# NVlabs/implicit_depth

Hardware: AMD Instinct MI355X
Metric: Mpoints/sec implicit-MLP query, 240x320x64 samples; depth L1 vs ref (higher is better)
Workload: dtype f32

## Files before the change

### implicit_depth_amd/csrc/lidf_api.hip

```cpp
#include <string.h>
#include <stdlib.h>

#include "lidf_launch.h"
#include "lidf_hip.h"

#define LIDF_API extern "C" __attribute__((visibility("default")))
#define CHECK_HIP(x)                       \
    do {                                   \
        if ((x) != hipSuccess) return LIDF_ERR_HIP; \
    } while (0)

static inline size_t align_up(size_t v, size_t a) { return (v + a - 1) / a * a; }
static size_t linex_stream_bytes(int k);

static hipError_t zero_words(void* a, size_t words_a, void* b, size_t words_b, hipStream_t st) {
    float* ptrs[2] = {(float*)a, (float*)b};
    const long long cnt[2] = {(long long)words_a, (long long)words_b};
    return lidf_launch_zero_segments(ptrs, cnt, 2, st);
}

static thread_local const LidfPackGuardState* tl_guard = nullptr;
struct GuardScope {
    explicit GuardScope(const LidfPackGuardState* g) { tl_guard = g; }
    ~GuardScope() { tl_guard = nullptr; }
};
static inline StreamLayout guarded(StreamLayout lay) {
    lay.guard = tl_guard;
    return lay;
}
static thread_local PackJobs* tl_jobs = nullptr;
static hipError_t flush_jobs(PackJobs& j, hipStream_t st) {
    const hipError_t e = lidf_launch_pack_multi(j, st);
    j.n = 0;
    return e;
}
static hipError_t pack_stream(const StreamLayout& lay, const NetW& n0, const NetW& n1, const L1Map& m,
                              float* stream, float* aux, hipStream_t st) {
    if (!tl_jobs) return lidf_launch_pack(guarded(lay), n0, n1, m, stream, aux, st);
    if (tl_jobs->n == LIDF_PACK_JOBS) {
        const hipError_t e = flush_jobs(*tl_jobs, st);
        if (e != hipSuccess) return e;
    }
    PackJob& k = tl_jobs->job[tl_jobs->n++];
    k.lay = guarded(lay); k.n0 = n0; k.n1 = n1; k.m = m; k.stream = stream; k.aux = aux;
    return hipSuccess;
}
struct JobScope {
    PackJobs jobs;
    JobScope() { jobs.n = 0; tl_jobs = &jobs; }
    ~JobScope() { tl_jobs = nullptr; }
};
static inline unsigned long long salt_mix(unsigned long long h, unsigned long long v) {
    h ^= v + 0x9E3779B97F4A7C15ull + (h << 6) + (h >> 2);
    h = (h ^ (h >> 30)) * 0xBF58476D1CE4E5B9ull;
    return h ^ (h >> 27);
}

static int cu_count(int* out) {
    int dev = 0;
    if (hipGetDevice(&dev) != hipSuccess) return LIDF_ERR_HIP;
    if (hipDeviceGetAttribute(out, hipDeviceAttributeMultiprocessorCount, dev) != hipSuccess)
        return LIDF_ERR_HIP;
    if (*out <= 0) *out = 256;
    return LIDF_OK;
}

static hipError_t zero_decoder_grads(const LidfDecoderGrads* g, int ld1, int is_ief, hipStream_t st) {
    float* const p[10] = {g->w1, g->b1, g->w2, g->b2, g->w3, g->b3, g->w4, g->b4,
                          is_ief ? g->wenc : nullptr, is_ief ? g->benc : nullptr};
    const long long c[10] = {(long long)LIDF_H1 * ld1, LIDF_H1, (long long)LIDF_H2 * LIDF_H1, LIDF_H2,
                             (long long)LIDF_H3 * LIDF_H2, LIDF_H3, LIDF_H3, 1, 16, 16};
    return lidf_launch_zero_segments(p, c, 10, st);
}

static int check_decoder(const LidfDecoder* d) {
    if (!d) return LIDF_OK;
    if (!d->w1 || !d->b1 || !d->w2 || !d->b2 || !d->w3 || !d->b3 || !d->w4 || !d->b4)
        return LIDF_ERR_BAD_ARG;
    if (d->is_ief && (!d->wenc || !d->benc || d->n_iter < 1 || d->n_iter > 64))
        return LIDF_ERR_BAD_ARG;
    return LIDF_OK;
}

static NetW to_netw(const LidfDecoder* d, int dcore) {
    NetW n;
    n.w1 = d->w1; n.b1 = d->b1; n.w2 = d->w2; n.b2 = d->b2;
    n.w3 = d->w3; n.b3 = d->b3; n.w4 = d->w4; n.b4 = d->b4;
    n.wenc = d->wenc; n.benc = d->benc;
    n.is_ief = d->is_ief ? 1 : 0;
    n.dcore = dcore;
    n.ld1 = dcore + (d->is_ief ? 16 : 0);
    return n;
}

static L1Map rows_map(int n0, int c0, int n1, int c1, int add_bias) {
    L1Map m = {};
    m.n0 = n0; m.c0 = c0; m.n1 = n1; m.c1 = c1;
    m.D = n0 + n1;
    m.KQ1 = (m.D + 1 + 7) / 8;
    m.add_bias = add_bias;
    m.nt = 8;
    m.nout = 256;
    return m;
}

static void fill_net_args(PointsArgs& a, int i, const LidfDecoder* d, float* out, int is_offset) {
    a.npass[i] = d->is_ief ? d->n_iter : 1;
    a.init[i] = d->is_ief ? d->init_offset : 0.f;
    a.sigmoid[i] = d->use_sigmoid;
    a.out[i] = out;
    a.is_offset[i] = is_offset;
}

LIDF_API int lidf_version(void) { return LIDF_ABI_VERSION; }

LIDF_API const char* lidf_strerror(int status) {
    switch (status) {
        case LIDF_OK: return "ok";
        case LIDF_ERR_BAD_ARG: return "lidf_hip: bad argument (null pointer, negative size or inconsistent sizes)";
        case LIDF_ERR_UNSUPPORTED: return "lidf_hip: unsupported dimension";
        case LIDF_ERR_WORKSPACE: return "lidf_hip: workspace too small";
        case LIDF_ERR_HIP: return "lidf_hip: HIP runtime error";
        default: return "lidf_hip: unknown status";
    }
}

LIDF_API int lidf_embed_f32(const float* x, int64_t n, int multires, float* out,
                              lidf_stream_t stream) {
    if (n < 0 || multires < 0 || multires > 16) return LIDF_ERR_BAD_ARG;
    if (n == 0) return LIDF_OK;
    if (!x || !out) return LIDF_ERR_BAD_ARG;
    CHECK_HIP(lidf_launch_embed(x, n, multires, out, (hipStream_t)stream));
    return LIDF_OK;
}

LIDF_API size_t lidf_decoders_workspace_bytes(int64_t n, int d) {
    (void)n;
    if (d <= 0) return 0;
    L1Map m = rows_map(d, 0, 0, 0, 1);
    StreamLayout lay = lidf_make_layout(2, LIDF_MODE_ROWS, m);
    const size_t hs = (size_t)lidf_make_layout_rows_h(2, d, 0).total * 4;
    const size_t fs = (size_t)lay.total * 4;
    return align_up(fs > hs ? fs : hs, 256) + align_up(2 * LIDF_AUX_FLOATS * 4, 256);
}

static int decoders_impl(const float* inp, int64_t n, int d, int64_t ld_inp, const LidfDecoder* prob,
                         const LidfDecoder* off, float* out_prob, float* out_off, void* workspace,
                         size_t workspace_bytes, int precision, lidf_stream_t stream,
                         const int* n_dev = nullptr);

LIDF_API int lidf_decoders_f32(const float* inp, int64_t n, int d, int64_t ld_inp,
                                 const LidfDecoder* prob, const LidfDecoder* off, float* out_prob,
                                 float* out_off, void* workspace, size_t workspace_bytes,
                                 lidf_stream_t stream) {
    return decoders_impl(inp, n, d, ld_inp, prob, off, out_prob, out_off, workspace, workspace_bytes,
// ... 2410 lines not shown
    if (!(voxpart_ready && pack_mode == 2) && (rc = run_linex(L, (float*)s_vox, cus, st, pack_mode))) return rc;
    if (make_raypart || pack_mode == 1) {
        LinEx Lr = {};
        Lr.w = off->w1; Lr.b = nullptr; Lr.ldw = ld1; Lr.nout = LIDF_H1;
        Lr.k = 128; Lr.c0 = 128;
        Lr.k1 = Ed; Lr.c1 = 256 + E;
        Lr.dcore = D;
        Lr.X = rayfeat; Lr.ldx = 128 + Ed; Lr.n = R; Lr.out = raypart; Lr.ld_out = LIDF_H1;
        Lr.n_dev = R_dev;
        if ((rc = run_linex(Lr, (float*)s_ray, cus, st, pack_mode))) return rc;
    }
    char* s16 = s_chain + chain_stream_bytes(D - 128);
    float* aux16 = (float*)(s16 + align_up(ief16_stream_bytes(3 + 6 * 16), 256));
    if (pack_mode != 2) {
        StreamLayout lay = {};
        lay.nets = 1; lay.mode = LIDF_MODE_IEF16;
        lay.total = (int)(ief16_stream_bytes(E) / 4);
        L1Map m16 = {};
        m16.n0 = E; m16.c0 = 256;
        const NetW nw = to_netw(off, D);
        CHECK_HIP(pack_stream(lay, nw, nw, m16, (float*)s16, aux16, st));
    }
    if (!use_ief16() || pack_mode == 1) {
        if (ev_rows && ev_rows[0] && pack_mode != 1) CHECK_HIP(hipEventRecord((hipEvent_t)ev_rows[0], st));
        rc = run_chain_train(off, D, rows_map(E, 256, 0, 0, 0), inp_embed ? inp_embed + 256 : nullptr, D, R,
                             end_voxel, nullptr, voxpart, raypart, nullptr, nullptr, out, s_chain, cus, st,
                             LIDF_MODE_ROWS_GATHER, pack_mode, R_dev);
        if (!rc && ev_rows && ev_rows[1] && pack_mode != 1) CHECK_HIP(hipEventRecord((hipEvent_t)ev_rows[1], st));
        return rc;
    }
    if (R <= 0) return LIDF_OK;
    if (ev_rows && ev_rows[0]) CHECK_HIP(hipEventRecord((hipEvent_t)ev_rows[0], st));
    Ief16Args ia = {};
    ia.stream = (const float*)s16; ia.aux = aux16; ia.KQ = (E + 15) / 16; ia.E = E;
    ia.n = R; ia.n_dev = R_dev;
    ia.X = inp_embed + 256; ia.ldx = D;
    ia.vox = end_voxel; ia.voxpart = voxpart; ia.raypart = raypart;
    ia.npass = off->is_ief ? off->n_iter : 1;
    ia.init = off->is_ief ? off->init_offset : 0.f;
    ia.sigmoid = off->use_sigmoid;
    ia.out = out;
    CHECK_HIP(lidf_launch_ief16(ia, cus, st));
    if (ev_rows && ev_rows[1]) CHECK_HIP(hipEventRecord((hipEvent_t)ev_rows[1], st));
    return LIDF_OK;
}

LIDF_API size_t lidf_refine_pack_bytes(int32_t multires, int32_t multires_views) {
    if (multires < 0 || multires > 16 || multires_views < 0 || multires_views > 16) return 0;
    return align_up(refine_fact_bytes(refine_D(multires, multires_views)), 256);
}

LIDF_API int lidf_refine_pack_f32(const LidfDecoder* off, int32_t multires, int32_t multires_views,
                                    void* packed, size_t packed_bytes, lidf_stream_t stream) {
    if (!off) return LIDF_ERR_BAD_ARG;
    int rc;
    if ((rc = check_decoder(off))) return rc;
    const size_t need = lidf_refine_pack_bytes(multires, multires_views);
    if (!need) return LIDF_ERR_UNSUPPORTED;
    if (!packed || packed_bytes < need) return LIDF_ERR_WORKSPACE;
    JobScope js;
    if ((rc = refine_pack_into(off, multires, multires_views, (char*)packed, (hipStream_t)stream))) return rc;
    CHECK_HIP(flush_jobs(js.jobs, (hipStream_t)stream));
    return LIDF_OK;
}

LIDF_API int lidf_refine_pack_guarded_f32(const LidfDecoder* off, int32_t multires,
                                            int32_t multires_views, void* packed, size_t packed_bytes,
                                            void* guard, lidf_stream_t stream) {
    if (!off || !guard) return LIDF_ERR_BAD_ARG;
    int rc;
    if ((rc = check_decoder(off))) return rc;
    const size_t need = lidf_refine_pack_bytes(multires, multires_views);
    if (!need) return LIDF_ERR_UNSUPPORTED;
    if (!packed || packed_bytes < need) return LIDF_ERR_WORKSPACE;
    const float* ptrs[LIDF_FP_MAX_SEGS];
    long long cnt[LIDF_FP_MAX_SEGS];
    const int k = decoder_segs(off, refine_D(multires, multires_views), ptrs, cnt, 0);
    return guarded_pack(ptrs, cnt, k, refine_salt(off, multires, multires_views), guard, (hipStream_t)stream, [&] {
        return lidf_refine_pack_f32(off, multires, multires_views, packed, packed_bytes, stream);
    });
}

struct TrainWs {
    size_t stream, dz1, dz2, dz3, S, goff, wg, chain, small, total;
};
static TrainWs train_ws(int64_t n, int d) {
    TrainWs w;
    const size_t N = (size_t)(n > 0 ? n : 1);
    size_t o = 0;
    const int kmax = d > 256 ? d : 256;
    w.stream = o; o += linex_stream_bytes(kmax);
    w.dz1 = o;    o += align_up(N * LIDF_H1 * 4, 256);
    w.dz2 = o;    o += align_up(N * LIDF_H2 * 4, 256);
    w.dz3 = o;    o += align_up(N * LIDF_H3 * 4, 256);
    w.S = o;      o += align_up(N * LIDF_H1 * 4, 256);
    w.goff = o;   o += align_up(N * 4, 256);
    w.wg = o;     o += align_up(WG_SCRATCH_FLOATS * 4, 256);
    w.chain = o;  o += chain_stream_bytes(d);
    w.small = o;  o += 512 * 4;
    w.total = o;
    return w;
}
LIDF_API size_t lidf_decoder_train_workspace_bytes(int64_t n, int32_t d) { return train_ws(n, d).total; }

static inline const unsigned* act_m1(const float* pass, int64_t n) { return (const unsigned*)(pass + (size_t)n * LIDF_ACT_M1); }
static inline const unsigned* act_m2(const float* pass, int64_t n) { return (const unsigned*)(pass + (size_t)n * LIDF_ACT_M2); }
static inline const float* act_h1(const float* act, int64_t n, int k) { return act + (size_t)k * n * ACT_ROW_FLOATS; }

LIDF_API int lidf_decoder_forward_train_f32(const float* inp, int64_t n, int32_t d, int64_t ld_inp,
                                              const LidfDecoder* dec, float* out, float* act,
                                              void* workspace, size_t workspace_bytes,
                                              lidf_stream_t stream) {
    if (n < 0 || d <= 0 || ld_inp < d || !dec) return LIDF_ERR_BAD_ARG;
    int rc;
    if ((rc = check_decoder(dec))) return rc;
    if (n == 0) return LIDF_OK;
    if (!inp || !out || !act) return LIDF_ERR_BAD_ARG;
    const TrainWs w = train_ws(n, d);
    if (!workspace || workspace_bytes < w.total) return LIDF_ERR_WORKSPACE;
    hipStream_t st = (hipStream_t)stream;
    float* sbuf = (float*)((char*)workspace + w.stream);
    int cus;
    if ((rc = cu_count(&cus))) return rc;
    const int npass = dec->is_ief ? dec->n_iter : 1;
    const int ld1 = d + (dec->is_ief ? 16 : 0);
    float* pre = act + (size_t)npass * n * ACT_ROW_FLOATS;
    (void)ld1; (void)sbuf;
    if ((rc = run_chain_train(dec, d, rows_map(d, 0, 0, 0, 1), inp, ld_inp, n, nullptr, nullptr, nullptr,
                              nullptr, act, pre, out, (char*)workspace + w.chain, cus, st)))
        return rc;
    return LIDF_OK;
}

static int decoder_backward_core(const float* inp, int64_t n, int32_t d, int64_t ld_inp, const LidfDecoder* dec,
                                 const float* act, const float* g_out, const LidfDecoderGrads* grads, char* ws,
                                 const TrainWs& w, int cus, hipStream_t st, float** S_out) {
    const int npass = dec->is_ief ? dec->n_iter : 1;
    const int ld1 = d + (dec->is_ief ? 16 : 0);
    float* sbuf = (float*)(ws + w.stream);
    float* dz1 = (float*)(ws + w.dz1);
    float* dz2 = (float*)(ws + w.dz2);
    float* dz3 = (float*)(ws + w.dz3);
    float* goff = (float*)(ws + w.goff);
    float* wgs = (float*)(ws + w.wg);
    const float* pre = act + (size_t)npass * n * ACT_ROW_FLOATS;
    float* S = (float*)(ws + w.S);
    float* small = (float*)(ws + w.small);
    CHECK_HIP(hipMemsetAsync(small, 0, 512 * 4, st));
    CHECK_HIP(lidf_launch_out_act(pre, n, dec->use_sigmoid, nullptr, g_out, goff, st));
    CHECK_HIP(lidf_launch_pack_dgrad(dec->w3, dec->w2, sbuf, st));
    if (npass == 1) S = dz1;
    for (int k = npass - 1; k >= 0; --k) {
        const float* h1 = act_h1(act, n, k);
        const float* h2 = h1 + (size_t)n * LIDF_H1;
        const float* h3 = h2 + (size_t)n * LIDF_H2;
        const float* offin = h3 + (size_t)n * LIDF_H3;
        CHECK_HIP(lidf_launch_l4_backward(goff, h3, dec->w4, 0.02f, n, dz3, grads->w4, grads->b4, wgs, st));
        CHECK_HIP(lidf_launch_wgrad(dz3, LIDF_H3, LIDF_H3, h2, LIDF_H2, LIDF_H2, n, grads->w3, LIDF_H2, grads->b3, wgs, WG_SCRATCH_FLOATS, st));
        const bool first_pass_short = dec->is_ief && npass > 1 && k == 0;
        float* dz1k = (k == npass - 1 || first_pass_short) ? S : dz1;
        CHECK_HIP(lidf_launch_dgrad_chain(nullptr, nullptr, dz3, act_m2(h1, n), act_m1(h1, n), n, 0.02f, dz2, dz1k,
                                          first_pass_short ? 1 : 0, sbuf, cus, st));
        CHECK_HIP(lidf_launch_wgrad(dz2, LIDF_H2, LIDF_H2, h1, LIDF_H1, LIDF_H1, n, grads->w2, LIDF_H1, grads->b2, wgs, WG_SCRATCH_FLOATS, st));
        if (dec->is_ief && !first_pass_short)
            CHECK_HIP(lidf_launch_ief_tail(dz1k, offin, dec->w1 + d, ld1, dec->wenc, dec->benc, n,
                                           k == npass - 1 ? 0 : 2, S, goff, grads->w1 + d, grads->wenc,
                                           grads->benc, npass > 1 ? small : nullptr, wgs, st));
    }
    CHECK_HIP(lidf_launch_wgrad(S, LIDF_H1, LIDF_H1, inp, ld_inp, d, n, grads->w1, ld1, grads->b1, wgs, WG_SCRATCH_FLOATS, st));
    if (dec->is_ief && npass > 1)
        CHECK_HIP(lidf_launch_ief_first_pass(grads->b1, small, dec->init_offset, dec->w1 + d, ld1, dec->wenc,
                                             dec->benc, grads->w1 + d, grads->wenc, grads->benc, st));
    *S_out = S;
    return LIDF_OK;
}

static int check_decoder_grads(const LidfDecoder* dec, const LidfDecoderGrads* grads) {
    if (!grads->w1 || !grads->b1 || !grads->w2 || !grads->b2 || !grads->w3 || !grads->b3 ||
        !grads->w4 || !grads->b4 || (dec->is_ief && (!grads->wenc || !grads->benc)))
        return LIDF_ERR_BAD_ARG;
    return LIDF_OK;
}

static int decoder_input_grad(const float* S, const LidfDecoder* dec, const float* S2, const LidfDecoder* dec2,
                              int64_t n, int32_t d, float* d_inp, int64_t ld_dinp, float* sbuf, int cus,
                              hipStream_t st) {
    LinEx L = {};
    L.n = n; L.transposed = 1; L.mask_slope = 0.02f;
    const int ld1 = d + (dec->is_ief ? 16 : 0);
    bool xcol = d % 32 == 1 && d > 32 && n > 16 * 128;
    if (xcol) {
        const int t = (d - 1) / 32, l = (t + 7) / 8;
        if ((t + l - 1) / l >= 8) xcol = false;
    }
    const int dt = xcol ? d - 1 : d;
    const int tiles = (dt + 31) / 32, launches = (tiles + 7) / 8, per = (tiles + launches - 1) / launches;
    for (int c0 = 0; c0 < dt; c0 += 32 * per) {
        int cols = dt - c0 < 32 * per ? dt - c0 : 32 * per;
        L.xcol = 0;
        if (xcol && c0 + cols == dt) { cols += 1; L.xcol = 1; }
        L.w = dec->w1 + c0; L.ldw = ld1; L.nout = cols; L.k = LIDF_H1; L.X = S; L.ldx = LIDF_H1;
        if (S2) {
            L.X2 = S2; L.ldx2 = LIDF_H1; L.k2 = LIDF_H1;
            L.w_2 = dec2->w1 + c0; L.ldw_2 = d + (dec2->is_ief ? 16 : 0);
        }
        L.out = d_inp + c0; L.ld_out = ld_dinp; L.accumulate = 0;
        int rc;
        if ((rc = run_linex(L, sbuf, cus, st))) return rc;
    }
    return LIDF_OK;
}

LIDF_API int lidf_decoder_backward_f32(const float* inp, int64_t n, int32_t d, int64_t ld_inp,
                                         const LidfDecoder* dec, const float* act,
                                         const float* g_out, float* d_inp, int64_t ld_dinp,
                                         const LidfDecoderGrads* grads, void* workspace,
                                         size_t workspace_bytes, lidf_stream_t stream) {
    if (n < 0 || d <= 0 || ld_inp < d || !dec || !grads) return LIDF_ERR_BAD_ARG;
    int rc;
    if ((rc = check_decoder(dec))) return rc;
    if ((rc = check_decoder_grads(dec, grads))) return rc;
    if (d_inp && ld_dinp < d) return LIDF_ERR_BAD_ARG;
    hipStream_t st = (hipStream_t)stream;
    CHECK_HIP(zero_decoder_grads(grads, d + (dec->is_ief ? 16 : 0), dec->is_ief, st));
    if (n == 0) return LIDF_OK;
    if (!inp || !act || !g_out) return LIDF_ERR_BAD_ARG;
    const TrainWs w = train_ws(n, d);
    if (!workspace || workspace_bytes < w.total) return LIDF_ERR_WORKSPACE;
    char* ws = (char*)workspace;
    int cus;
    if ((rc = cu_count(&cus))) return rc;
    float* S = nullptr;
    if ((rc = decoder_backward_core(inp, n, d, ld_inp, dec, act, g_out, grads, ws, w, cus, st, &S))) return rc;
    if (d_inp) return decoder_input_grad(S, dec, nullptr, nullptr, n, d, d_inp, ld_dinp, (float*)(ws + w.stream), cus, st);
    return LIDF_OK;
}

LIDF_API size_t lidf_decoder_pair_workspace_bytes(int64_t n, int32_t d) {
    return 2 * align_up(train_ws(n, d).total, 256) + linex_stream_bytes(2 * LIDF_H1);
}
LIDF_API size_t lidf_decoder_pair_workspace_offset(int64_t n, int32_t d, int32_t which) {
    return (size_t)(which ? 1 : 0) * align_up(train_ws(n, d).total, 256);
}

LIDF_API int lidf_decoder_pair_backward_f32(const float* inp, int64_t n, int32_t d, int64_t ld_inp,
                                              const LidfDecoder* prob, const LidfDecoder* off,
                                              const float* act_prob, const float* act_off,
                                              const float* g_prob, const float* g_off, float* d_inp,
                                              int64_t ld_dinp, const LidfDecoderGrads* grads_prob,
                                              const LidfDecoderGrads* grads_off, void* workspace,
                                              size_t workspace_bytes, lidf_stream_t stream) {
    if (n < 0 || d <= 0 || ld_inp < d || !prob || !off || !grads_prob || !grads_off) return LIDF_ERR_BAD_ARG;
    int rc;
    if ((rc = check_decoder(prob)) || (rc = check_decoder(off))) return rc;
    if ((rc = check_decoder_grads(prob, grads_prob)) || (rc = check_decoder_grads(off, grads_off))) return rc;
    if (d_inp && ld_dinp < d) return LIDF_ERR_BAD_ARG;
    hipStream_t st = (hipStream_t)stream;
    CHECK_HIP(zero_decoder_grads(grads_prob, d + (prob->is_ief ? 16 : 0), prob->is_ief, st));
    CHECK_HIP(zero_decoder_grads(grads_off, d + (off->is_ief ? 16 : 0), off->is_ief, st));
    if (n == 0) return LIDF_OK;
    if (!inp || !act_prob || !act_off || !g_prob || !g_off) return LIDF_ERR_BAD_ARG;
    const TrainWs w = train_ws(n, d);
    const size_t one = align_up(w.total, 256);
    if (!workspace || workspace_bytes < lidf_decoder_pair_workspace_bytes(n, d)) return LIDF_ERR_WORKSPACE;
    char* ws = (char*)workspace;
    int cus;
    if ((rc = cu_count(&cus))) return rc;
    float *Sp = nullptr, *So = nullptr;
    if ((rc = decoder_backward_core(inp, n, d, ld_inp, prob, act_prob, g_prob, grads_prob, ws, w, cus, st, &Sp))) return rc;
    if ((rc = decoder_backward_core(inp, n, d, ld_inp, off, act_off, g_off, grads_off, ws + one, w, cus, st, &So))) return rc;
    if (d_inp) return decoder_input_grad(Sp, prob, So, off, n, d, d_inp, ld_dinp, (float*)(ws + 2 * one), cus, st);
    return LIDF_OK;
}

LIDF_API int lidf_build_rows_f32(const int32_t* pair_ray, const int32_t* pair_vox,
                                   const float* pair_t, const float* ray_dir,
                                   const float* vox_center, int32_t pos_rel, const float* vox_feat,
                                   const float* rayfeat, int32_t multires, int32_t multires_views,
                                   int64_t n_pairs, float* rows, lidf_stream_t stream) {
    if (n_pairs < 0 || multires < 0 || multires > 16 || multires_views < 0 || multires_views > 16)
        return LIDF_ERR_BAD_ARG;
    if (n_pairs == 0) return LIDF_OK;
    if (!pair_ray || !pair_vox || !pair_t || !ray_dir || !vox_feat || !rayfeat || !rows)
        return LIDF_ERR_BAD_ARG;
    if (pos_rel && !vox_center) return LIDF_ERR_BAD_ARG;
    const int Ed = 3 + 6 * multires_views;
    CHECK_HIP(lidf_launch_build_rows(pair_ray, pair_vox, pair_t, ray_dir, vox_center, pos_rel,
                                     vox_feat, rayfeat, 128 + Ed, multires, Ed, n_pairs, rows,
                                     query_D(multires, multires_views), (hipStream_t)stream));
    return LIDF_OK;
}

LIDF_API int lidf_rows_backward_f32(const float* d_rows, const int32_t* pair_off,
                                      const int32_t* pair_vox, int64_t n_rays, int64_t n_pairs,
                                      int64_t n_vox, int32_t multires, int32_t multires_views,
                                      float* d_vox_feat, float* d_rayfeat, lidf_stream_t stream) {
    if (n_pairs < 0 || n_rays < 0 || n_vox < 0 || multires < 0 || multires > 16 ||
        multires_views < 0 || multires_views > 16)
        return LIDF_ERR_BAD_ARG;
    hipStream_t st = (hipStream_t)stream;
    const int E = 3 + 6 * multires, Ed = 3 + 6 * multires_views;
    if (d_vox_feat && n_vox > 0) CHECK_HIP(hipMemsetAsync(d_vox_feat, 0, (size_t)n_vox * 128 * 4, st));
    if (n_rays == 0) return LIDF_OK;
    if (!pair_off || (n_pairs > 0 && (!d_rows || !pair_vox))) return LIDF_ERR_BAD_ARG;
    CHECK_HIP(lidf_launch_rows_backward(d_rows, query_D(multires, multires_views), 2 * E, pair_off, pair_vox, n_rays,
                                        n_pairs, Ed, d_vox_feat, d_rayfeat, 128 + Ed, st));
    return LIDF_OK;
}

LIDF_API int lidf_ray_features_backward_f32(const float* d_rayfeat, const int32_t* ray_pix,
                                              const int32_t* ray_bid, int64_t n_rays, int32_t batch,
                                              int32_t height, int32_t width, int32_t roi_inp_bbox,
                                              int32_t multires_views, float* d_feat_grid,
                                              void* workspace, size_t workspace_bytes,
                                              lidf_stream_t stream) {
    if (n_rays < 0 || batch <= 0 || height <= 0 || width <= 0 || !d_feat_grid) return LIDF_ERR_BAD_ARG;
    hipStream_t st = (hipStream_t)stream;
    CHECK_HIP(hipMemsetAsync(d_feat_grid, 0, (size_t)batch * 32 * height * width * 4, st));
    if (n_rays == 0) return LIDF_OK;
    if (!d_rayfeat || !ray_pix || !ray_bid) return LIDF_ERR_BAD_ARG;
    const size_t need = (size_t)batch * 128 * height * width * 4;
    const size_t need2 = need + (size_t)batch * height * width * 4;
    float* gimg = (workspace && workspace_bytes >= need) ? (float*)workspace : nullptr;
    int* pix_rays = (workspace && workspace_bytes >= need2) ? (int*)((char*)workspace + need) : nullptr;
    CHECK_HIP(lidf_launch_rayfeat_backward(d_rayfeat, 128 + 3 + 6 * multires_views, ray_pix, ray_bid,
                                           n_rays, roi_inp_bbox / 2, batch, height, width, d_feat_grid,
                                           gimg, pix_rays, st));
    return LIDF_OK;
}

LIDF_API int lidf_pe_rows_f32(const int32_t* pair_ray, const int32_t* pair_vox, const float* pair_t,
                                const float* ray_dir, const float* vox_center, int32_t pos_rel,
                                int32_t multires, int64_t n_pairs, float* pe, lidf_stream_t stream) {
    if (n_pairs < 0 || multires < 0 || multires > 16) return LIDF_ERR_BAD_ARG;
    if (n_pairs == 0) return LIDF_OK;
    if (!pair_ray || !pair_vox || !pair_t || !ray_dir || !pe || (pos_rel && !vox_center))
        return LIDF_ERR_BAD_ARG;
    if (n_pairs * 2 * (3 + 6 * multires) > 0x7fffffffLL * 256) return LIDF_ERR_UNSUPPORTED;
    CHECK_HIP(lidf_launch_pe_rows(pair_ray, pair_vox, pair_t, ray_dir, vox_center, pos_rel, multires,
                                  n_pairs, pe, (hipStream_t)stream));
    return LIDF_OK;
}

static inline size_t qact_pass(int64_t P) { return (size_t)P * ACT_ROW_FLOATS; }

LIDF_API size_t lidf_query_decoder_act_floats(int64_t n_pairs, int64_t n_rays, int64_t n_vox,
                                                int32_t n_pass) {
    if (n_pairs < 0 || n_rays < 0 || n_vox < 0 || n_pass <= 0) return 0;
    return (size_t)(n_vox + n_rays) * LIDF_H1 + (size_t)n_pass * qact_pass(n_pairs) + (size_t)n_pairs;
}

struct QTrainWs {
    size_t stream, dz1, dz2, dz3, S, goff, dvox, dray, wg, seg, seg_bytes, chain, small, total;
};
static QTrainWs qtrain_ws(int64_t P, int64_t R, int64_t V) {
    QTrainWs w;
    const size_t N = (size_t)(P > 0 ? P : 1);
    size_t o = 0;
    w.stream = o; o += linex_stream_bytes(256);
    w.dz1 = o;    o += align_up(N * LIDF_H1 * 4, 256);
    w.dz2 = o;    o += align_up(N * LIDF_H2 * 4, 256);
    w.dz3 = o;    o += align_up(N * LIDF_H3 * 4, 256);
    w.S = o;      o += align_up(N * LIDF_H1 * 4, 256);
    w.goff = o;   o += align_up(N * 4, 256);
    w.dvox = o;   o += align_up((size_t)(V > 0 ? V : 1) * LIDF_H1 * 4, 256);
    w.dray = o;   o += align_up((size_t)(R > 0 ? R : 1) * LIDF_H1 * 4, 256);
    w.wg = o;     o += align_up(WG_SCRATCH_FLOATS * 4, 256);
    w.seg_bytes = lidf_seg_sum_idx_ws_bytes(P, V);
    w.seg = o;    o += align_up(w.seg_bytes, 256);
    w.chain = o;  o += chain_stream_bytes(2 * (3 + 6 * 16));
    w.small = o;  o += 512 * 4;
    w.total = o;
    return w;
}
LIDF_API size_t lidf_query_decoder_workspace_bytes(int64_t n_pairs, int64_t n_rays, int64_t n_vox) {
    return qtrain_ws(n_pairs, n_rays, n_vox).total;
}

static int check_qtrain(const LidfQueryTrainArgs* q) {
    if (!q || !q->dec) return LIDF_ERR_BAD_ARG;
    if (q->n_pairs < 0 || q->n_rays < 0 || q->n_vox < 0) return LIDF_ERR_BAD_ARG;
    if (q->multires < 0 || q->multires > 16 || q->multires_views < 0 || q->multires_views > 16)
        return LIDF_ERR_BAD_ARG;
    if (q->n_pairs > 0 && (!q->pair_off || !q->pair_ray || !q->pair_vox || !q->pe || !q->vox_feat ||
                           !q->rayfeat || q->n_rays == 0 || q->n_vox == 0))
        return LIDF_ERR_BAD_ARG;
    return check_decoder(q->dec);
}

static int qdec_forward_impl(const LidfQueryTrainArgs* q, int E2, float* out, float* voxpart, float* raypart,
                             float* passes, float* pre, float* s_vox, float* s_ray, char* s_chain, int cus,
                             hipStream_t st, int pack_mode = 0, int parts = 7, int pe_ld = 0) {
    int rc;
    const int64_t P = q->n_pairs, R = q->n_rays, V = q->n_vox;
    const LidfDecoder* dec = q->dec;
    const int Ed = 3 + 6 * q->multires_views;
    const int D = 256 + E2 + Ed, ld1 = D + (dec->is_ief ? 16 : 0);
    LinEx L = {};
    if (parts & 1) {
        L.w = dec->w1; L.b = dec->b1; L.ldw = ld1; L.nout = LIDF_H1; L.k = 128; L.dcore = D;
        L.ief = dec->is_ief ? dec : nullptr;
        L.X = q->vox_feat; L.ldx = 128; L.n = V; L.out = voxpart; L.ld_out = LIDF_H1;
        if ((rc = run_linex(L, s_vox, cus, st, pack_mode))) return rc;
    }
    if (parts & 2) {
        L = {};
        L.w = dec->w1; L.ldw = ld1; L.nout = LIDF_H1; L.k = 128; L.c0 = 128; L.k1 = Ed; L.c1 = 256 + E2;
        L.X = q->rayfeat; L.ldx = 128 + Ed; L.n = R; L.out = raypart; L.ld_out = LIDF_H1;
        if ((rc = run_linex(L, s_ray, cus, st, pack_mode))) return rc;
    }
    if (parts & 4) {
        if ((rc = run_chain_train(dec, D, rows_map(E2, 256, 0, 0, 0), q->pe, pe_ld ? pe_ld : E2, P, q->pair_vox,
                                  q->pair_ray, voxpart, raypart, passes, pre, out, s_chain, cus, st, LIDF_MODE_TRAIN,
                                  pack_mode)))
            return rc;
    }
    return LIDF_OK;
}

LIDF_API int lidf_query_decoder_forward_train_f32(const LidfQueryTrainArgs* q, float* out, float* act,
                                                    void* workspace, size_t workspace_bytes,
                                                    lidf_stream_t stream) {
    int rc;
    if ((rc = check_qtrain(q))) return rc;
    const int64_t P = q->n_pairs, R = q->n_rays, V = q->n_vox;
    if (P == 0) return LIDF_OK;
    if (!out || !act) return LIDF_ERR_BAD_ARG;
    const QTrainWs w = qtrain_ws(P, R, V);
    if (!workspace || workspace_bytes < w.total) return LIDF_ERR_WORKSPACE;
    hipStream_t st = (hipStream_t)stream;
    float* sbuf = (float*)((char*)workspace + w.stream);
    int cus;
    if ((rc = cu_count(&cus))) return rc;
    const LidfDecoder* dec = q->dec;
    const int E2 = 2 * (3 + 6 * q->multires);
    const int npass = dec->is_ief ? dec->n_iter : 1;
    float* voxpart = act;
    float* raypart = voxpart + (size_t)V * LIDF_H1;
    float* passes = raypart + (size_t)R * LIDF_H1;
    float* pre = passes + (size_t)npass * qact_pass(P);
    return qdec_forward_impl(q, E2, out, voxpart, raypart, passes, pre, sbuf, sbuf, (char*)workspace + w.chain,
                             cus, st);
}

LIDF_API size_t lidf_query_forward_train_workspace_bytes(int64_t n_rays, int64_t n_vox) {
    return lidf_query_workspace_bytes(n_rays, n_vox, 0);
}

LIDF_API int lidf_query_forward_train_f32(const LidfQueryTrainArgs* q, const LidfDecoder* offset_dec,
                                            const float* pair_t, const float* ray_dir,
                                            const float* vox_center, int32_t pos_rel, float* out_prob,
                                            float* out_off, float* act_prob, float* act_off,
                                            void* workspace, size_t workspace_bytes,
                                            lidf_stream_t stream) {
    int rc;
    if ((rc = check_qtrain(q))) return rc;
    if ((rc = check_decoder(offset_dec))) return rc;
    const int64_t P = q->n_pairs, R = q->n_rays, V = q->n_vox;
    if (P > 0x7fffffffLL || R > 0x15555555LL) return LIDF_ERR_UNSUPPORTED;
    const int L = q->multires, Lv = q->multires_views;
    if ((rc = check_query_model(q->dec, offset_dec, L, Lv, LIDF_PRECISION_F32))) return rc;
    if (P == 0) return LIDF_OK;
    if (!pair_t || !ray_dir || !out_prob || !out_off || !act_prob || !act_off || (pos_rel && !vox_center))
        return LIDF_ERR_BAD_ARG;
    const QueryWs w = query_ws(R, V, L, Lv);
    if (!workspace || workspace_bytes < w.total) return LIDF_ERR_WORKSPACE;
    hipStream_t st = (hipStream_t)stream;
    char* ws = (char*)workspace;
    const QueryPlan p = query_plan(L, Lv, LIDF_PRECISION_F32);
    if ((rc = pack_query_weights(q->dec, offset_dec, p, ws, st))) return rc;
    int cus;
    if ((rc = cu_count(&cus))) return rc;
    CHECK_HIP(lidf_launch_l1only_pair(
        l1_table_args(p, L1_RAY, q->rayfeat, R, nullptr, (float*)(ws + w.raypart), ws, w),
        l1_table_args(p, L1_VOX, q->vox_feat, V, nullptr, (float*)(ws + w.voxpart), ws, w), nullptr, cus, st));
    PointsArgs a = points_args(p, ws, ws, w, P, q->pair_ray, q->pair_vox, pair_t, ray_dir, vox_center, pos_rel,
                               0.f, 0.f, 0.f);
    fill_net_args(a, 0, q->dec, out_prob, 0);
    fill_net_args(a, 1, offset_dec, out_off, 1);
    const LidfDecoder* decs[2] = {q->dec, offset_dec};
    float* acts[2] = {act_prob, act_off};
    for (int i = 0; i < 2; ++i) {
        const int np = decs[i]->is_ief ? decs[i]->n_iter : 1;
        a.tr_passes[i] = acts[i] + (size_t)(V + R) * LIDF_H1;
        a.tr_pre[i] = a.tr_passes[i] + (size_t)np * qact_pass(P);
    }
    a.tr_pass_floats = (long long)qact_pass(P);
    const long long nt = (P + 127) / 128;
    CHECK_HIP(lidf_launch_points(LIDF_MODE_FUSED, a, (int)(nt < cus ? nt : cus), st));
    return LIDF_OK;
}

LIDF_API int lidf_query_forward_train_selected_f32(const LidfQueryTrainArgs* q, const LidfDecoder* offset_dec,
                                                     const float* pair_t, const float* ray_dir,
                                                     const float* vox_center, int32_t pos_rel, float offset_range0,
                                                     float offset_range1, float part_size,
                                                     const int64_t* max_pair_id_in, float* out_prob, float* softmax,
                                                     int64_t* max_pair_id, float* pred_offset, float* pair_pred_pos,
                                                     float* pred_pos, float* act_prob, float* act_off_rows,
                                                     void* workspace, size_t workspace_bytes, lidf_stream_t stream) {
    int rc;
    if ((rc = check_qtrain(q))) return rc;
    if ((rc = check_decoder(offset_dec))) return rc;
    const int64_t P = q->n_pairs, R = q->n_rays, V = q->n_vox;
    if (P > 0x7fffffffLL || R > 0x15555555LL) return LIDF_ERR_UNSUPPORTED;
    const int L = q->multires, Lv = q->multires_views;
    if ((rc = check_query_model(q->dec, offset_dec, L, Lv, LIDF_PRECISION_F32))) return rc;
    if (R == 0) return LIDF_OK;
    if (!max_pair_id || !pred_pos) return LIDF_ERR_BAD_ARG;
    hipStream_t st = (hipStream_t)stream;
    if (P == 0) {
        CHECK_HIP(lidf_launch_ray_reduce_dev(nullptr, nullptr, q->pair_off, R, 0, nullptr, nullptr, nullptr, nullptr, 0,
                                             nullptr, (long long*)max_pair_id, pred_pos, nullptr, st, nullptr, nullptr,
                                             nullptr, nullptr, nullptr));
        return LIDF_OK;
    }
    if (!pair_t || !ray_dir || !out_prob || !softmax || !pred_offset || !pair_pred_pos || !act_prob || !act_off_rows ||
        (pos_rel && !vox_center))
        return LIDF_ERR_BAD_ARG;
    const QueryWs w = query_ws(R, V, L, Lv);
    if (!workspace || workspace_bytes < w.total) return LIDF_ERR_WORKSPACE;
    char* ws = (char*)workspace;
    const QueryPlan p = query_plan(L, Lv, LIDF_PRECISION_F32);
    if ((rc = pack_query_weights(q->dec, offset_dec, p, ws, st))) return rc;
    int cus;
    if ((rc = cu_count(&cus))) return rc;
    CHECK_HIP(lidf_launch_l1only_pair(
        l1_table_args(p, L1_RAY, q->rayfeat, R, nullptr, (float*)(ws + w.raypart), ws, w),
        l1_table_args(p, L1_VOX, q->vox_feat, V, nullptr, (float*)(ws + w.voxpart), ws, w), nullptr, cus, st));
    PointsArgs a = points_args(p, ws, ws, w, P, q->pair_ray, q->pair_vox, pair_t, ray_dir, vox_center, pos_rel,
                               offset_range0, offset_range1, part_size);
    a.nets = 1; a.part_ld = 512; a.part_off = 0;
    fill_net_args(a, 0, q->dec, out_prob, 0);
    a.tr_passes[0] = act_prob + (size_t)(V + R) * LIDF_H1;
    a.tr_pre[0] = a.tr_passes[0] + qact_pass(P);
    a.tr_pass_floats = (long long)qact_pass(P);
    const long long nt = (P + 127) / 128;
    CHECK_HIP(lidf_launch_points(LIDF_MODE_FUSED, a, (int)(nt < cus ? nt : cus), st));
    const SelList sl = sel_list(ws + w.sel, R);
    const bool given = max_pair_id_in != nullptr;
    CHECK_HIP(lidf_launch_ray_reduce_dev(out_prob, nullptr, q->pair_off, R, P, nullptr, nullptr, nullptr, nullptr, 0,
                                         softmax, (long long*)max_pair_id, nullptr, nullptr, st, q->pair_vox, pair_t,
                                         given ? nullptr : sl.ray, sl.vox, sl.t));
    if (given)
        CHECK_HIP(lidf_launch_sel_from_ids((const long long*)max_pair_id_in, q->pair_vox, pair_t, R, P, sl.ray, sl.vox,
                                           sl.t, st));
    const int npo = offset_dec->is_ief ? offset_dec->n_iter : 1;
    PointsArgs ao = offset_on_list(a, p, offset_dec, sl, R);
    ao.tr_passes[0] = act_off_rows + (size_t)(V + R) * LIDF_H1;
    ao.tr_pre[0] = ao.tr_passes[0] + (size_t)npo * qact_pass(R);
    ao.tr_pass_floats = (long long)qact_pass(R);
    const long long ntr = (R + 127) / 128;
    CHECK_HIP(lidf_launch_points(LIDF_MODE_FUSED, ao, (int)(ntr < cus ? ntr : cus), st));
    CHECK_HIP(lidf_launch_selected_finish((const long long*)(given ? max_pair_id_in : max_pair_id), sl.off, sl.pos, R, P,
                                          nullptr, nullptr, nullptr, nullptr, 0, pred_offset, pair_pred_pos, pred_pos,
                                          nullptr, st));
    return LIDF_OK;
}

struct QdecBwd {
    int E2;
    bool zero_grads;
    float* S_keep;
    float* d_pe;
    float *s_dvox, *s_dpe;
    int pack_mode;
    const float* s_dgrad;
    bool goff_ready;
    const float* l1rows;
    int l1_ld, l1_cols, l1_c0;
    const int *ss_perm, *ss_vstart, *ss_first;
    long long ss_row0, ss_n;
    float* ss_partial;
};
static int qdec_backward_impl(const LidfQueryTrainArgs* q, const QdecBwd& o, const float* passes, const float* pre,
                              const float* g_out, float* d_vox_feat, float* d_rayfeat, int accumulate_inputs,
                              const LidfDecoderGrads* grads, char* ws, const QTrainWs& w, int cus, hipStream_t st) {
    int rc;
    const LidfDecoder* dec = q->dec;
    const int64_t P = q->n_pairs, R = q->n_rays, V = q->n_vox;
    const int E2 = o.E2, Ed = 3 + 6 * q->multires_views;
    const int D = 256 + E2 + Ed, ld1 = D + (dec->is_ief ? 16 : 0);
    const int npass = dec->is_ief ? dec->n_iter : 1;
    float* sbuf = (float*)(ws + w.stream);
    float* dz1 = (float*)(ws + w.dz1);
    float* dz2 = (float*)(ws + w.dz2);
    float* dz3 = (float*)(ws + w.dz3);
    float* S = o.S_keep ? o.S_keep : (float*)(ws + w.S);
    float* goff = (float*)(ws + w.goff);
    float* wgs = (float*)(ws + w.wg);
    float* dvox = (float*)(ws + w.dvox);
    float* dray = (float*)(ws + w.dray);
    float* small = (float*)(ws + w.small);
    CHECK_HIP(hipMemsetAsync(small, 0, 512 * 4, st));
    if (!o.goff_ready) CHECK_HIP(lidf_launch_out_act(pre, P, dec->use_sigmoid, nullptr, g_out, goff, st));
    const float* dgs = o.s_dgrad;
    if (!dgs) {
        CHECK_HIP(lidf_launch_pack_dgrad(dec->w3, dec->w2, sbuf, st));
        dgs = sbuf;
    }
    for (int k = npass - 1; k >= 0; --k) {
        const float* h1 = passes + (size_t)k * qact_pass(P);
        const float* h2 = h1 + (size_t)P * LIDF_H1;
        const float* h3 = h2 + (size_t)P * LIDF_H2;
        const float* offin = h3 + (size_t)P * LIDF_H3;
        CHECK_HIP(lidf_launch_l4_backward(goff, h3, dec->w4, 0.02f, P, dz3, grads->w4, grads->b4, wgs, st));
        CHECK_HIP(lidf_launch_wgrad(dz3, LIDF_H3, LIDF_H3, h2, LIDF_H2, LIDF_H2, P, grads->w3, LIDF_H2, grads->b3, wgs, WG_SCRATCH_FLOATS, st));
        if (npass == 1) {
            if (o.S_keep) dz1 = S;
            else S = dz1;
        }
        const bool first_pass_short = dec->is_ief && npass > 1 && k == 0;
        float* dz1k = (k == npass - 1 || first_pass_short) ? S : dz1;
        CHECK_HIP(lidf_launch_dgrad_chain(nullptr, nullptr, dz3, act_m2(h1, P), act_m1(h1, P), P, 0.02f, dz2, dz1k,
                                          first_pass_short ? 1 : 0, (float*)dgs, cus, st));
        CHECK_HIP(lidf_launch_wgrad(dz2, LIDF_H2, LIDF_H2, h1, LIDF_H1, LIDF_H1, P, grads->w2, LIDF_H1, grads->b2, wgs, WG_SCRATCH_FLOATS, st));
        if (!first_pass_short)
            CHECK_HIP(lidf_launch_ief_tail(dz1k, offin, dec->is_ief ? dec->w1 + D : nullptr, ld1, dec->wenc,
                                           dec->benc, P, k == npass - 1 ? 0 : 2, S, goff,
                                           grads->w1 + D, grads->wenc, grads->benc,
                                           dec->is_ief && npass > 1 ? small : nullptr, wgs, st));
    }
    const bool short_first = dec->is_ief && npass > 1;
    if (o.l1rows)
        CHECK_HIP(lidf_launch_wgrad(S, LIDF_H1, LIDF_H1, o.l1rows, o.l1_ld, o.l1_cols, P, grads->w1 + o.l1_c0, ld1,
                                    short_first ? small + 256 : nullptr, wgs, WG_SCRATCH_FLOATS, st));
    else
        CHECK_HIP(lidf_launch_wgrad(S, LIDF_H1, LIDF_H1, q->pe, E2, E2, P, grads->w1 + 256, ld1,
                                    short_first ? small + 256 : nullptr, wgs, WG_SCRATCH_FLOATS, st));
    if (short_first)
        CHECK_HIP(lidf_launch_ief_first_pass(small + 256, small, dec->init_offset, dec->w1 + D, ld1,
                                             dec->wenc, dec->benc, grads->w1 + D, grads->wenc,
                                             grads->benc, st));
    if (o.ss_perm)
        CHECK_HIP(lidf_launch_pnet_gather_segsum(S, o.ss_perm, o.ss_row0, o.ss_vstart, o.ss_first, V, o.ss_n,
                                                 o.ss_partial, dvox, st));
    else
        CHECK_HIP(lidf_launch_seg_sum_idx(S, q->pair_vox, P, V, dvox, w.seg_bytes ? ws + w.seg : nullptr,
                                          w.seg_bytes, st));
    CHECK_HIP(lidf_launch_wgrad(dvox, LIDF_H1, LIDF_H1, q->vox_feat, 128, 128, V, grads->w1, ld1, grads->b1, wgs, WG_SCRATCH_FLOATS, st));
    if (!o.S_keep) {
        CHECK_HIP(lidf_launch_seg_sum_ray(S, LIDF_H1, q->pair_off, R, dray, st));
        CHECK_HIP(lidf_launch_wgrad(dray, LIDF_H1, LIDF_H1, q->rayfeat, 128 + Ed, 128, R, grads->w1 + 128, ld1, nullptr, wgs, WG_SCRATCH_FLOATS, st));
        CHECK_HIP(lidf_launch_wgrad(dray, LIDF_H1, LIDF_H1, q->rayfeat + 128, 128 + Ed, Ed, R, grads->w1 + 256 + E2, ld1, nullptr, wgs, WG_SCRATCH_FLOATS, st));
    }
    LinEx L = {};
    L.transposed = 1; L.ldw = ld1; L.k = LIDF_H1; L.ldx = LIDF_H1; L.accumulate = accumulate_inputs ? 1 : 0;
    if (d_vox_feat) {
        L.w = dec->w1; L.nout = 128; L.X = dvox; L.n = V; L.out = d_vox_feat; L.ld_out = 128;
        if ((rc = run_linex(L, o.s_dvox ? o.s_dvox : sbuf, cus, st, o.s_dvox ? o.pack_mode : 0))) return rc;
    }
    if (o.d_pe) {
        L.w = dec->w1 + 256; L.nout = E2; L.X = S; L.n = P; L.out = o.d_pe; L.ld_out = E2; L.accumulate = 0;
        if ((rc = run_linex(L, o.s_dpe ? o.s_dpe : sbuf, cus, st, o.s_dpe ? o.pack_mode : 0))) return rc;
        L.accumulate = accumulate_inputs ? 1 : 0;
    }
    if (d_rayfeat && !o.S_keep) {
        L.w = dec->w1 + 128; L.nout = 128; L.X = dray; L.n = R; L.out = d_rayfeat; L.ld_out = 128 + Ed;
        if ((rc = run_linex(L, sbuf, cus, st))) return rc;
        L.w = dec->w1 + 256 + E2; L.nout = Ed; L.out = d_rayfeat + 128;
        if ((rc = run_linex(L, sbuf, cus, st))) return rc;
    }
    return LIDF_OK;
}

LIDF_API int lidf_query_decoder_backward_f32(const LidfQueryTrainArgs* q, const float* act,
                                               const float* g_out, float* d_vox_feat,
                                               float* d_rayfeat, int32_t accumulate_inputs,
                                               const LidfDecoderGrads* grads, void* workspace,
                                               size_t workspace_bytes, lidf_stream_t stream) {
    int rc;
    if ((rc = check_qtrain(q))) return rc;
    if (!grads) return LIDF_ERR_BAD_ARG;
    const LidfDecoder* dec = q->dec;
    if (!grads->w1 || !grads->b1 || !grads->w2 || !grads->b2 || !grads->w3 || !grads->b3 ||
        !grads->w4 || !grads->b4 || (dec->is_ief && (!grads->wenc || !grads->benc)))
        return LIDF_ERR_BAD_ARG;
    const int64_t P = q->n_pairs, R = q->n_rays, V = q->n_vox;
    hipStream_t st = (hipStream_t)stream;
    const int E2 = 2 * (3 + 6 * q->multires), Ed = 3 + 6 * q->multires_views;
    const int D = 256 + E2 + Ed, ld1 = D + (dec->is_ief ? 16 : 0);
    const int npass = dec->is_ief ? dec->n_iter : 1;
    CHECK_HIP(zero_decoder_grads(grads, ld1, dec->is_ief, st));
    if (!accumulate_inputs) {
        if (d_vox_feat && V > 0) CHECK_HIP(hipMemsetAsync(d_vox_feat, 0, (size_t)V * 128 * 4, st));
        if (d_rayfeat && R > 0) CHECK_HIP(hipMemsetAsync(d_rayfeat, 0, (size_t)R * (128 + Ed) * 4, st));
    }
    if (P == 0) return LIDF_OK;
    if (!act || !g_out) return LIDF_ERR_BAD_ARG;
    const QTrainWs w = qtrain_ws(P, R, V);
    if (!workspace || workspace_bytes < w.total) return LIDF_ERR_WORKSPACE;
    int cus;
    if ((rc = cu_count(&cus))) return rc;
    const float* voxpart = act;
    const float* raypart = voxpart + (size_t)V * LIDF_H1;
    const float* passes = raypart + (size_t)R * LIDF_H1;
    const float* pre = passes + (size_t)npass * qact_pass(P);
    QdecBwd o = {};
    o.E2 = E2; o.zero_grads = true;
    return qdec_backward_impl(q, o, passes, pre, g_out, d_vox_feat, d_rayfeat, accumulate_inputs, grads,
                              (char*)workspace, w, cus, st);
}

struct QRowsWs { size_t pvox, poff, g, pe, act, inner, total; QTrainWs w; };
static QRowsWs qrows_ws(int64_t R, int64_t V, int E2, int npass) {
    QRowsWs l;
    const size_t N = (size_t)(R > 0 ? R : 1);
    size_t o = 0;
    l.pvox = o;  o += align_up(N * 4, 256);
    l.poff = o;  o += align_up((N + 1) * 4, 256);
    l.g = o;     o += align_up(N * 4, 256);
    l.pe = o;    o += align_up(N * (size_t)E2 * 4, 256);
    l.act = o;   o += align_up(((size_t)npass * qact_pass((int64_t)N) + N) * 4, 256);
    l.w = qtrain_ws(R, R, V);
    l.inner = o; o += l.w.total;
    l.total = o;
    return l;
}
LIDF_API size_t lidf_query_decoder_rows_workspace_bytes(int64_t n_rays, int64_t n_vox, int32_t multires,
                                                          int32_t n_pass) {
    if (n_rays < 0 || n_vox < 0 || multires < 0 || multires > 16 || n_pass <= 0) return 0;
    return qrows_ws(n_rays, n_vox, 2 * (3 + 6 * multires), n_pass).total;
}
LIDF_API int lidf_query_decoder_backward_rows_f32(const LidfQueryTrainArgs* q, const float* act, int32_t act_is_rows,
                                                    const int64_t* rows, const float* g_pred_pos,
                                                    const float* g_offset_rows, const float* ray_dir, float scale,
                                                    float* d_vox_feat,
                                                    float* d_rayfeat, int32_t accumulate_inputs,
                                                    const LidfDecoderGrads* grads, void* workspace,
                                                    size_t workspace_bytes, lidf_stream_t stream) {
    int rc;
    if ((rc = check_qtrain(q))) return rc;
    if (!grads) return LIDF_ERR_BAD_ARG;
    const LidfDecoder* dec = q->dec;
    if (!grads->w1 || !grads->b1 || !grads->w2 || !grads->b2 || !grads->w3 || !grads->b3 ||
        !grads->w4 || !grads->b4 || (dec->is_ief && (!grads->wenc || !grads->benc)))
        return LIDF_ERR_BAD_ARG;
    const int64_t P = q->n_pairs, R = q->n_rays, V = q->n_vox;
    hipStream_t st = (hipStream_t)stream;
    const int E2 = 2 * (3 + 6 * q->multires), Ed = 3 + 6 * q->multires_views;
    const int D = 256 + E2 + Ed, ld1 = D + (dec->is_ief ? 16 : 0);
    const int npass = dec->is_ief ? dec->n_iter : 1;
    CHECK_HIP(zero_decoder_grads(grads, ld1, dec->is_ief, st));
    if (!accumulate_inputs) {
        if (d_vox_feat && V > 0) CHECK_HIP(hipMemsetAsync(d_vox_feat, 0, (size_t)V * 128 * 4, st));
        if (d_rayfeat && R > 0) CHECK_HIP(hipMemsetAsync(d_rayfeat, 0, (size_t)R * (128 + Ed) * 4, st));
    }
    if (P == 0 || R == 0) return LIDF_OK;
    if (!act || !rows || !ray_dir) return LIDF_ERR_BAD_ARG;
    const QRowsWs l = qrows_ws(R, V, E2, npass);
    if (!workspace || workspace_bytes < l.total) return LIDF_ERR_WORKSPACE;
    int cus;
    if ((rc = cu_count(&cus))) return rc;
    char* ws = (char*)workspace;
    int* pvox = (int*)(ws + l.pvox);
    int* poff = (int*)(ws + l.poff);
    float* g = (float*)(ws + l.g);
    float* pe = (float*)(ws + l.pe);
    const float* passes_src = act + (size_t)(V + R) * LIDF_H1;
    const float* passes = act_is_rows ? passes_src : (const float*)(ws + l.act);
    CHECK_HIP(lidf_launch_gather_sel_rows(act_is_rows ? nullptr : passes_src, P, npass, (const long long*)rows, R,
                                          q->pair_vox, q->pe, E2, g_pred_pos, g_offset_rows, ray_dir, scale,
                                          (float*)(ws + l.act), pvox, pe, g, poff, st));
    LidfQueryTrainArgs qc = *q;
    qc.n_pairs = R;
    qc.pair_off = poff; qc.pair_ray = poff; qc.pair_vox = pvox; qc.pe = pe;
    QdecBwd o = {};
    o.E2 = E2; o.zero_grads = true;
    return qdec_backward_impl(&qc, o, passes, passes + (size_t)npass * qact_pass(R), g, d_vox_feat, d_rayfeat,
                              accumulate_inputs, grads, ws + l.inner, l.w, cus, st);
}

LIDF_API int lidf_query_tail_f32(const float* pred_offset, const float* pred_prob,
                                   const int32_t* pair_off, const int32_t* pair_ray,
                                   const float* pair_t, const float* ray_dir, int64_t n_rays,
                                   int64_t n_pairs, float offset_range0, float offset_range1,
                                   float part_size, const int64_t* max_pair_id_in,
                                   float* pair_pred_pos, float* softmax, int64_t* max_pair_id,
                                   float* pred_pos, lidf_stream_t stream) {
    if (n_rays < 0 || n_pairs < 0) return LIDF_ERR_BAD_ARG;
    if (n_rays == 0) return LIDF_OK;
    if (!pair_off || (n_pairs > 0 && (!pred_offset || !pred_prob || !pair_ray || !pair_t || !ray_dir ||
                                      !pair_pred_pos)))
        return LIDF_ERR_BAD_ARG;
    hipStream_t st = (hipStream_t)stream;
    CHECK_HIP(lidf_launch_pair_pos(pred_offset, pair_ray, pair_t, ray_dir, n_pairs, offset_range0,
                                   offset_range1 - offset_range0, (float)1.7320508075688772,
                                   part_size, pair_pred_pos, st));
    CHECK_HIP(lidf_launch_ray_reduce(pred_prob, pair_pred_pos, pair_off, n_rays, n_pairs, nullptr,
                                     nullptr, 0, softmax, (long long*)max_pair_id,
                                     max_pair_id_in ? nullptr : pred_pos, nullptr, st));
    if (max_pair_id_in && pred_pos)
        CHECK_HIP(lidf_launch_ray_select(pair_pred_pos, (const long long*)max_pair_id_in, n_rays,
                                         n_pairs, pred_pos, st));
    return LIDF_OK;
}

LIDF_API int lidf_query_tail_backward_f32(const float* g_pair_pred_pos, const float* g_pred_pos,
                                            const int64_t* max_pair_id, const int32_t* pair_ray,
                                            const float* ray_dir, int64_t n_rays, int64_t n_pairs,
                                            float offset_range0, float offset_range1,
                                            float part_size, float* d_pred_offset,
                                            lidf_stream_t stream) {
    if (n_rays < 0 || n_pairs < 0) return LIDF_ERR_BAD_ARG;
    if (n_pairs == 0) return LIDF_OK;
    if (!pair_ray || !ray_dir || !d_pred_offset || (g_pred_pos && !max_pair_id)) return LIDF_ERR_BAD_ARG;
    const float k = (offset_range1 - offset_range0) * (float)1.7320508075688772 * part_size;
    CHECK_HIP(lidf_launch_pair_pos_backward(g_pair_pred_pos, g_pred_pos, (const long long*)max_pair_id,
                                            pair_ray, ray_dir, n_pairs, k, d_pred_offset,
                                            (hipStream_t)stream));
    return LIDF_OK;
}

LIDF_API int lidf_embed_backward_f32(const float* x, const float* g_out, int64_t n, int multires,
                                       float* d_x, lidf_stream_t stream) {
    if (n < 0 || multires < 0 || multires > 16) return LIDF_ERR_BAD_ARG;
    if (n == 0) return LIDF_OK;
    if (!x || !g_out || !d_x) return LIDF_ERR_BAD_ARG;
    CHECK_HIP(lidf_launch_embed_backward(x, g_out, n, multires, d_x, (hipStream_t)stream));
    return LIDF_OK;
}

struct PnetAct {
    size_t f1, f2, f4, f5, pool1, g1, pool2, out, arg1, arg2, total;
};
static PnetAct pnet_act(int64_t n, int64_t v) {
    PnetAct a;
    const size_t N = (size_t)(n > 0 ? n : 1), V = (size_t)(v > 0 ? v : 1);
    size_t o = 0;
    a.f1 = o; o += N * 32;
    a.f2 = o; o += N * 64;
    a.f4 = o; o += N * 128;
    a.f5 = o; o += N * 128;
// ... 492 lines not shown
```

### implicit_depth_amd/csrc/lidf_api_refine_train.inc

```

struct RtLay {
    size_t s_pnf[7], s_pnb[PNET_BWD_SLOTS], s_pnchain, s_pnbwd, s_vox, s_ray, s_chain, s_dvox, s_dpe, s_dgrad;
    size_t raypart, ray_idx, iter0, iter_bytes, total;
    size_t cur, end_voxel, pn_inp, pn_vox, pnact, pe, voxpart, passes, pre, off;
};
static RtLay rt_lay(int64_t R, int64_t Nv, int64_t V, int E, int npass, int T) {
    RtLay l;
    size_t o = 0;
    const int ks[7] = {6, 32, 64, 64, 64, 128, 128};
    const int nts[7] = {1, 2, 2, 4, 4, 4, 4};
    for (int i = 0; i < 7; ++i) { l.s_pnf[i] = o; o += lin_stream_bytes(ks[i], nts[i]); }
    for (int i = 0; i < PNET_BWD_SLOTS; ++i) { l.s_pnb[i] = o; o += linex_stream_bytes(PNET_BWD_SLOT_K[i]); }
    l.s_pnchain = o; o += align_up(lidf_pointnet_chain_stream_bytes(), 256);
    l.s_pnbwd = o;   o += align_up(PNETC_BWD_STREAM_BYTES, 256);
    l.s_vox = o;   o += linex_stream_bytes(128);
    l.s_ray = o;   o += linex_stream_bytes(REFINE_RAY_K);
    l.s_chain = o; o += chain_stream_bytes(3 + 6 * 16);
    l.s_dvox = o;  o += linex_stream_bytes(256);
    l.s_dpe = o;   o += linex_stream_bytes(256);
    l.s_dgrad = o; o += align_up(lidf_dgrad_stream_bytes(), 256);
    const size_t r = (size_t)(R > 0 ? R : 1), n = (size_t)(R + Nv > 0 ? R + Nv : 1), v = (size_t)(V > 0 ? V : 1);
    l.raypart = o; o += align_up(r * LIDF_H1 * 4, 256);
    l.ray_idx = o; o += align_up(r * 4, 256);
    l.iter0 = o;
// ... 89 lines not shown
    }
    if (nc > 0x7fffffffLL) return LIDF_ERR_UNSUPPORTED;
    cells->g.crop = q->grid_part;
    cells->g.B = q->batch;
    cells->coord = q->voxel_coord;
    cells->table = q->cell_table;
    cells->ready = q->cell_table_ready;
    return LIDF_OK;
}

static int rt_pack_transposed(const LidfDecoder* dec, int E, int Ed, float* s_dvox, float* s_dpe, int cus,
                              hipStream_t st) {
    int rc;
    const int D = 256 + E + Ed, ld1 = D + (dec->is_ief ? 16 : 0);
    LinEx L = {};
    L.transposed = 1; L.ldw = ld1; L.k = LIDF_H1; L.ldx = LIDF_H1;
    L.w = dec->w1; L.nout = 128; L.ld_out = 128;
    if ((rc = run_linex(L, s_dvox, cus, st, 1))) return rc;
    L.w = dec->w1 + 256; L.nout = E; L.ld_out = E;
    return run_linex(L, s_dpe, cus, st, 1);
}

static void rt_query_args(const LidfRefineArgs* q, const RtLay& l, char* it, char* act, LidfQueryTrainArgs* t) {
    *t = {};
    t->n_pairs = q->n_rays; t->n_rays = q->n_rays; t->n_vox = q->n_vox;
    t->pair_off = nullptr;
    t->pair_ray = (const int32_t*)(act + l.ray_idx);
    t->pair_vox = (const int32_t*)(it + l.end_voxel);
    t->pe = (const float*)(it + l.pe) + 128;
    t->multires = q->multires; t->multires_views = q->multires_views;
    const int64_t n = q->n_rays + q->n_valid;
    t->vox_feat = pnetc_ok(n, q->n_vox) ? (const float*)(it + l.pnact + pnetc_act(n, q->n_vox).out)
                                        : (const float*)(it + l.pnact) + pnet_act(n, q->n_vox).out;
    t->rayfeat = q->rayfeat;
    t->dec = q->off;
}

LIDF_API int lidf_refine_train_forward_f32(const LidfRefineArgs* q, int32_t forward_times, void* act_v,
                                             size_t act_bytes, lidf_stream_t stream) {
    int rc, cus;
    const int T = forward_times;
    if ((rc = rt_check(q, T))) return rc;
    const int64_t R = q->n_rays, Nv = q->n_valid, V = q->n_vox, P = q->n_pairs, n = R + Nv;
    if (R == 0) return LIDF_OK;
    const LidfDecoder* dec = q->off;
    const int E = 3 + 6 * q->multires, Ed = 3 + 6 * q->multires_views;
    const int npass = dec->is_ief ? dec->n_iter : 1;
    const RtLay l = rt_lay(R, Nv, V, E, npass, T);
    const RtWs w = rt_ws(R, Nv, V, E);
    if (!act_v || act_bytes < l.total) return LIDF_ERR_WORKSPACE;
    if (!q->workspace || q->workspace_bytes < w.total) return LIDF_ERR_WORKSPACE;
    CellLookup cells;
    if ((rc = rt_cells(q, &cells))) return rc;
    if ((rc = cu_count(&cus))) return rc;
    hipStream_t st = (hipStream_t)stream;
    char* act = (char*)act_v;
    char* ws = (char*)q->workspace;
    const bool chain = pnetc_ok(n, V);
    float* pnf[7];
    float* pnb[PNET_BWD_SLOTS];
    for (int i = 0; i < 7; ++i) pnf[i] = (float*)(act + l.s_pnf[i]);
    for (int i = 0; i < PNET_BWD_SLOTS; ++i) pnb[i] = (float*)(act + l.s_pnb[i]);
    float* raypart = (float*)(act + l.raypart);
    int* ray_idx = (int*)(act + l.ray_idx);
    LidfQueryTrainArgs t;
    rt_query_args(q, l, act + l.iter0, act, &t);
    {
        JobScope js;
        if (chain)
            rc = pnetc_pack(q->pnet, (float*)(act + l.s_pnchain), pnf, (float*)(act + l.s_pnbwd), cus, st);
        else
            rc = pointnet_train_forward_impl(q->pnet, nullptr, nullptr, 0, 0, nullptr,
                                             (float*)(act + l.iter0 + l.pnact), nullptr, pnf, cus, st, 1);
        if (!rc) {
            LidfPointNetGrads none = {};
            rc = pointnet_backward_impl(q->pnet, nullptr, nullptr, 0, 0, (const float*)(act + l.iter0 + l.pnact),
                                        nullptr, nullptr, &none, ws + w.pn, w.pw, false, pnb, 1, cus, st);
        }
        if (!rc)
            rc = qdec_forward_impl(&t, E, nullptr, nullptr, nullptr, nullptr, nullptr, (float*)(act + l.s_vox),
                                   (float*)(act + l.s_ray), act + l.s_chain, cus, st, 1);
        if (!rc)
            rc = rt_pack_transposed(dec, E, Ed, (float*)(act + l.s_dvox), (float*)(act + l.s_dpe), cus, st);
        if (!rc && flush_jobs(js.jobs, st) != hipSuccess) rc = LIDF_ERR_HIP;
        if (rc) return rc;
    }
    CHECK_HIP(lidf_launch_pack_dgrad(dec->w3, dec->w2, (float*)(act + l.s_dgrad), st));
    CHECK_HIP(lidf_launch_iota(ray_idx, R, st));
    if ((rc = qdec_forward_impl(&t, E, nullptr, nullptr, raypart, nullptr, nullptr, nullptr, (float*)(act + l.s_ray),
                                nullptr, cus, st, 2, 2)))
        return rc;
    const float r0 = q->offset_range0, rs = q->offset_range1 - q->offset_range0;
    const float* cur = q->pred_pos;
    for (int it = 0; it < T; ++it) {
        char* ib = act + l.iter0 + (size_t)it * l.iter_bytes;
        float* cur_keep = (float*)(ib + l.cur);
        int* end_voxel = (int*)(ib + l.end_voxel);
        char* pib = chain ? act + l.iter0 : ib;
        float* pn_inp = (float*)(pib + l.pn_inp);
        int* pn_vox = (int*)(pib + l.pn_vox);
        float* pnact = (float*)(ib + l.pnact);
        float* pe = (float*)(ib + l.pe);
        float* off = (float*)(ib + l.off);
        const PnetAct pa = pnet_act(n, V);
        if (it == 0) {
            CHECK_HIP(hipMemcpyAsync(cur_keep, cur, (size_t)R * 12, hipMemcpyDeviceToDevice, st));
            cur = cur_keep;
        }
        if (Nv > 0 && (!chain || it == 0)) {
            CHECK_HIP(hipMemcpyAsync(pn_inp, q->valid_inp, (size_t)Nv * 24, hipMemcpyDeviceToDevice, st));
            CHECK_HIP(hipMemcpyAsync(pn_vox, q->valid_vox, (size_t)Nv * 4, hipMemcpyDeviceToDevice, st));
        }
        cells.ready = q->cell_table_ready || it > 0;
        CHECK_HIP(lidf_launch_refine_prep(cur, (const long long*)q->max_pair_id, q->pair_vox, P, q->voxel_bound,
                                          q->voxel_bid, V, q->ray_bid, q->ray_flat, q->rgb_img,
                                          (long long)q->height * q->width, q->rayfeat, 128 + Ed, q->multires_views,
                                          q->multires, q->pnet_pos_rel, q->pos_rel, R, pn_inp + (size_t)Nv * 6,
                                          pn_vox + Nv, nullptr, 0, end_voxel, nullptr, st,
                                          q->voxel_coord ? &cells : nullptr));
        CHECK_HIP(lidf_launch_refine_rows_dev(cur, end_voxel, q->voxel_bound, q->rayfeat, 128 + Ed, q->multires_views,
                                              q->multires, q->pos_rel, R, nullptr, pe - 128, 128 + E + Ed, 0, st));
        if (chain)
            rc = pnetc_forward(pn_inp, pn_vox, n, V, nullptr, (char*)pnact, ws + w.pn,
                               (const float*)(act + l.s_pnchain), pnf, cus, st);
        else
            rc = pointnet_train_forward_impl(q->pnet, pn_inp, pn_vox, n, V, pnact + pa.out, pnact,
                                             (float*)(ws + w.pn + w.pw.gpart), pnf, cus, st, 2);
        if (rc) return rc;
        rt_query_args(q, l, ib, act, &t);
        if ((rc = qdec_forward_impl(&t, E, off, (float*)(ib + l.voxpart), raypart, (float*)(ib + l.passes),
                                    (float*)(ib + l.pre), (float*)(act + l.s_vox), nullptr, act + l.s_chain, cus, st,
                                    2, 1 | 4, 128 + E + Ed)))
            return rc;
        float* out = it == T - 1 ? q->pred_pos_out : (float*)(ib + l.iter_bytes + l.cur);
        CHECK_HIP(lidf_launch_refine_finish(cur, off, q->ray_dir, r0, rs, R, out, st));
        if (it == T - 1 && q->end_voxel_id)
            CHECK_HIP(hipMemcpyAsync(q->end_voxel_id, end_voxel, (size_t)R * 4, hipMemcpyDeviceToDevice, st));
        cur = out;
    }
    return LIDF_OK;
}

LIDF_API int lidf_refine_train_backward_f32(const LidfRefineArgs* q, int32_t forward_times, const void* act_v,
                                              size_t act_bytes, const float* g_pos, float* d_pred_pos,
                                              float* d_rayfeat, const LidfPointNetGrads* gp,
                                              const LidfDecoderGrads* gd, lidf_stream_t stream) {
    int rc, cus;
    const int T = forward_times;
    if ((rc = rt_check(q, T, false))) return rc;
    if (!gp || !gd) return LIDF_ERR_BAD_ARG;
    const LidfDecoder* dec = q->off;
    if (!gd->w1 || !gd->b1 || !gd->w2 || !gd->b2 || !gd->w3 || !gd->b3 || !gd->w4 || !gd->b4 ||
        (dec->is_ief && (!gd->wenc || !gd->benc)))
        return LIDF_ERR_BAD_ARG;
    if (!gp->w_p1 || !gp->b_p1 || !gp->w_p2 || !gp->b_p2 || !gp->w_v1 || !gp->b_v1 || !gp->w_p3 || !gp->b_p3 ||
        !gp->w_p4 || !gp->b_p4 || !gp->w_v2 || !gp->b_v2)
        return LIDF_ERR_BAD_ARG;
    const int64_t R = q->n_rays, Nv = q->n_valid, V = q->n_vox, n = R + Nv;
    const int E = 3 + 6 * q->multires, Ed = 3 + 6 * q->multires_views;
    const int D = refine_D(q->multires, q->multires_views), ld1 = D + (dec->is_ief ? 16 : 0);
    const int npass = dec->is_ief ? dec->n_iter : 1;
    hipStream_t st = (hipStream_t)stream;
    CHECK_HIP(zero_decoder_grads(gd, ld1, dec->is_ief, st));
    {
        float* const zp[12] = {gp->w_p1, gp->b_p1, gp->w_p2, gp->b_p2, gp->w_v1, gp->b_v1, gp->w_p3, gp->b_p3,
                               gp->w_p4, gp->b_p4, gp->w_v2, gp->b_v2};
        const long long zc[12] = {32 * 6, 32, 64 * 32, 64, 64 * 64, 64, 128 * 128, 128, 128 * 128, 128, 128 * 128, 128};
        CHECK_HIP(lidf_launch_zero_segments(zp, zc, 12, st));
    }
    if (R == 0) return LIDF_OK;
    if (!g_pos) return LIDF_ERR_BAD_ARG;
    const RtLay l = rt_lay(R, Nv, V, E, npass, T);
    const RtWs w = rt_ws(R, Nv, V, E);
    if (!act_v || act_bytes < l.total) return LIDF_ERR_WORKSPACE;
    if (!q->workspace || q->workspace_bytes < w.total) return LIDF_ERR_WORKSPACE;
    if ((rc = cu_count(&cus))) return rc;
    const bool chain = pnetc_ok(n, V);
    char* act = (char*)act_v;
    char* ws = (char*)q->workspace;
    float* pnb[PNET_BWD_SLOTS];
    for (int i = 0; i < PNET_BWD_SLOTS; ++i) pnb[i] = (float*)(act + l.s_pnb[i]);
    float* ssum = (float*)(ws + w.ssum);
    float* s_it = (float*)(ws + w.s_it);
    float* dvoxfeat = (float*)(ws + w.dvoxfeat);
    float* d_pe = (float*)(ws + w.d_pe);
    float* d_inp = (float*)(ws + w.d_inp);
    float* gbuf[2] = {(float*)(ws + w.g_a), (float*)(ws + w.g_b)};
    float* goff_in = (float*)(ws + w.goff_in);
    float* wgs = (float*)(ws + w.qd + w.qw.wg);
    const float rs = q->offset_range1 - q->offset_range0;
    const float* g = g_pos;
    const PnetAct pa = pnet_act(n, V);
    for (int it = T - 1; it >= 0; --it) {
        char* ib = act + l.iter0 + (size_t)it * l.iter_bytes;
        const float* cur = (const float*)(ib + l.cur);
        const int* end_voxel = (const int*)(ib + l.end_voxel);
        const float* pnact = (const float*)(ib + l.pnact);
        const bool need_dcur = it > 0 || d_pred_pos != nullptr;
        CHECK_HIP(lidf_launch_refine_train_goff(g, q->ray_dir, rs, R, (const float*)(ib + l.pre), dec->use_sigmoid,
                                                (float*)(ws + w.qd + w.qw.goff), st));
        (void)goff_in;
        LidfQueryTrainArgs t;
        rt_query_args(q, l, ib, act, &t);
        QdecBwd o = {};
        o.E2 = E; o.zero_grads = false;
        o.S_keep = (d_rayfeat && it == T - 1) ? ssum : s_it;
        o.l1rows = (const float*)(ib + l.pe); o.l1_ld = 128 + E + Ed; o.l1_cols = 128 + E + Ed; o.l1_c0 = 128;
        o.d_pe = need_dcur ? d_pe : nullptr;
        o.s_dvox = (float*)(act + l.s_dvox); o.s_dpe = (float*)(act + l.s_dpe); o.pack_mode = 2;
        o.s_dgrad = (const float*)(act + l.s_dgrad);
        o.goff_ready = true;
        if (chain) {
            const PnetActC pc = pnetc_act(n, V);
            size_t sc_off, perm_off;
            int nblk;
            lidf_sort_idx_layout(n, V, &sc_off, &nblk, &perm_off);
            const char* pb = (const char*)pnact;
            o.ss_perm = (const int*)(pb + pc.sort + perm_off);
            o.ss_vstart = (const int*)(pb + pc.vstart);
            o.ss_first = (const int*)(pb + pc.first);
            o.ss_row0 = Nv; o.ss_n = n;
            o.ss_partial = (float*)(ws + w.ss_partial);
        }
        if ((rc = qdec_backward_impl(&t, o, (const float*)(ib + l.passes), (const float*)(ib + l.pre), goff_in,
                                     dvoxfeat, nullptr, 0, gd, ws + w.qd, w.qw, cus, st)))
            return rc;
        if (d_rayfeat && it != T - 1) CHECK_HIP(lidf_launch_add_inplace(ssum, s_it, R * LIDF_H1, st));
        if (chain)
            rc = pnetc_backward(q->pnet, n, V, (const char*)pnact, dvoxfeat, need_dcur ? d_inp : nullptr, true, gp,
                                ws + w.pn, pnb, 2, (const float*)(act + l.s_pnbwd), cus, st);
        else
            rc = pointnet_backward_impl(q->pnet, (const float*)(ib + l.pn_inp), (const int32_t*)(ib + l.pn_vox), n, V,
                                        pnact, dvoxfeat, need_dcur ? d_inp : nullptr, gp, ws + w.pn, w.pw, false, pnb,
                                        2, cus, st);
        if (rc) return rc;
        (void)pa;
        if (need_dcur) {
            float* gn = it == 0 ? d_pred_pos : gbuf[it & 1];
            CHECK_HIP(lidf_launch_refine_train_dcur(g, cur, end_voxel, q->voxel_bound, q->pos_rel, d_pe, q->multires,
                                                    d_inp + (size_t)Nv * 6, R, gn, st));
            g = gn;
        }
    }
    (void)wgs;
    if (d_rayfeat) {
        float* sbuf = (float*)(ws + w.qd + w.qw.stream);
        LinEx L = {};
        L.transposed = 1; L.ldw = ld1; L.k = LIDF_H1; L.ldx = LIDF_H1; L.X = ssum; L.n = R;
        L.w = dec->w1 + 128; L.nout = 128; L.out = d_rayfeat; L.ld_out = 128 + Ed;
        if ((rc = run_linex(L, sbuf, cus, st))) return rc;
        L.w = dec->w1 + 256 + E; L.nout = Ed; L.out = d_rayfeat + 128;
        if ((rc = run_linex(L, sbuf, cus, st))) return rc;
    }
    return LIDF_OK;
}

static long long rstep_n_cells(int32_t batch, const int32_t* grid_res) {
    if (!grid_res || batch <= 0) return 0;
    long long nc = batch;
    for (int k = 0; k < 3; ++k) {
        if (grid_res[k] <= 0) return 0;
        nc *= grid_res[k];
        if (nc > 0x7fffffffLL) return -1;
    }
    return nc;
}

LIDF_API size_t lidf_refine_step_workspace_bytes(int32_t batch, const int32_t* grid_res) {
    const long long nc = rstep_n_cells(batch, grid_res);
    return nc > 0 ? (size_t)nc * 4 : 0;
}

LIDF_API int lidf_refine_step_forward_f32(const float* pos, const int64_t* max_pair_id, const int32_t* pair_vox,
                                            int64_t n_pairs, const float* voxel_bound, const int32_t* voxel_bid,
                                            int64_t n_vox, const int32_t* ray_bid, const int32_t* ray_flat,
                                            const float* rgb_img, int32_t batch, int32_t height, int32_t width,
                                            int64_t n_rays, int64_t n_valid, int32_t pnet_pos_rel, int32_t pos_rel,
                                            int32_t multires, const int32_t* voxel_coord, const int32_t* grid_res,
                                            const float* grid_xmin, float grid_part, int32_t cell_table_ready,
                                            int32_t* end_voxel, float* pnet_inp, int32_t* pnet_vox, float* pe,
                                            int64_t ld_pe, void* workspace, size_t workspace_bytes,
                                            lidf_stream_t stream) {
    if (n_rays < 0 || n_pairs < 0 || n_vox < 0 || n_valid < 0 || multires < 0 || multires > 16)
        return LIDF_ERR_BAD_ARG;
    if (n_rays == 0) return LIDF_OK;
    if (n_vox == 0 || batch <= 0 || height <= 0 || width <= 0 || ld_pe < 3 + 6 * multires) return LIDF_ERR_BAD_ARG;
    if (!pos || !max_pair_id || !voxel_bound || !voxel_bid || !ray_bid || !ray_flat || !rgb_img || !end_voxel ||
        !pnet_inp || !pnet_vox || !pe || (n_pairs > 0 && !pair_vox))
        return LIDF_ERR_BAD_ARG;
    if (((uintptr_t)pos | (uintptr_t)pnet_inp | (uintptr_t)pe) & 3) return LIDF_ERR_BAD_ARG;
    if (n_rays + n_valid > 0x15555555LL || n_vox > 0x7fffffffLL || n_pairs > 0x7fffffffLL) return LIDF_ERR_UNSUPPORTED;
    CellLookup cells = {};
    if (voxel_coord) {
        const long long nc = rstep_n_cells(batch, grid_res);
        if (nc == 0 || !grid_xmin || !(grid_part > 0.f)) return LIDF_ERR_BAD_ARG;
        if (nc < 0) return LIDF_ERR_UNSUPPORTED;
        if (!workspace || workspace_bytes < (size_t)nc * 4) return LIDF_ERR_WORKSPACE;
        for (int k = 0; k < 3; ++k) {
            cells.g.xmin[k] = grid_xmin[k];
            cells.g.r[k] = grid_res[k];
        }
        cells.g.crop = grid_part;
        cells.g.B = batch;
        cells.coord = voxel_coord;
        cells.table = (int*)workspace;
        cells.ready = cell_table_ready;
    }
    RayStepArgs a = {};
    a.pos = pos; a.max_pair_id = (const long long*)max_pair_id; a.pair_vox = pair_vox;
    a.R = n_rays; a.P = n_pairs; a.V = n_vox; a.n_valid = n_valid;
    a.vbound = voxel_bound; a.vox_bid = voxel_bid; a.ray_bid = ray_bid; a.ray_flat = ray_flat;
    a.rgb = rgb_img; a.hw = (long long)height * width;
    a.pnet_rel = pnet_pos_rel ? 1 : 0; a.pos_rel = pos_rel ? 1 : 0; a.L = multires;
    a.end_voxel = end_voxel; a.pnet_inp = pnet_inp; a.pnet_vox = pnet_vox; a.pe = pe; a.ld_pe = ld_pe;
    CHECK_HIP(lidf_launch_refine_raystep(a, voxel_coord ? &cells : nullptr, (hipStream_t)stream));
    return LIDF_OK;
}

LIDF_API int lidf_refine_step_backward_f32(const float* g_pos, const float* ray_dir, float offset_range0,
                                             float offset_range1, float* d_off, const float* pos,
                                             const int32_t* end_voxel, const float* voxel_bound, int32_t pos_rel,
                                             const float* d_pe, int32_t multires, const float* d_pnet_rows,
                                             float* d_pos, int64_t n_rays, lidf_stream_t stream) {
    if (n_rays < 0 || multires < 0 || multires > 16) return LIDF_ERR_BAD_ARG;
    if (n_rays == 0 || (!d_off && !d_pos)) return LIDF_OK;
    if (!g_pos || (d_off && !ray_dir)) return LIDF_ERR_BAD_ARG;
    if (d_pos && d_pe && (!pos || (pos_rel && (!end_voxel || !voxel_bound)))) return LIDF_ERR_BAD_ARG;
    if (n_rays > 0x15555555LL) return LIDF_ERR_UNSUPPORTED;
    hipStream_t st = (hipStream_t)stream;
    if (d_off)
        CHECK_HIP(lidf_launch_refine_train_goff(g_pos, ray_dir, offset_range1 - offset_range0, n_rays, nullptr, 0,
                                                d_off, st));
    if (d_pos)
        CHECK_HIP(lidf_launch_refine_train_dcur(g_pos, pos, end_voxel, voxel_bound, pos_rel ? 1 : 0, d_pe, multires,
                                                d_pnet_rows, n_rays, d_pos, st));
// ... 3 lines not shown
```

### implicit_depth_amd/csrc/lidf_device.h

```cpp
#pragma once
#include <hip/hip_runtime.h>
#include <stdint.h>

#if defined(__HIP_DEVICE_COMPILE__) && !defined(__gfx950__) && !defined(__gfx942__)
#error "liblidf_hip orders its ticket reductions by returned atomic values (gfx942/gfx950 behaviour); use release/acquire on other targets"
#endif

typedef float f32x16 __attribute__((ext_vector_type(16)));
typedef float f32x4 __attribute__((ext_vector_type(4)));
typedef float f32x2 __attribute__((ext_vector_type(2)));
typedef float f32x4u __attribute__((ext_vector_type(4), aligned(4)));

#define LIDF_H1 256
#define LIDF_H2 128
#define LIDF_H3 64
#define LIDF_ACT_OIN (LIDF_H1 + LIDF_H2 + LIDF_H3)
#define LIDF_ACT_M1 (LIDF_ACT_OIN + 1)
#define LIDF_ACT_M2 (LIDF_ACT_M1 + 8)
#define LIDF_ACT_ROW_FLOATS (LIDF_ACT_M2 + 4)
#define LIDF_WG_SLAB (128 * 256 + 512)
#define LIDF_RING 8
#define LIDF_L2_QUADS 33
#define LIDF_L3_QUADS 17
#define LIDF_U_QUADS 2
#define LIDF_PASS_QUADS (LIDF_U_QUADS + 4 * LIDF_L2_QUADS + 2 * LIDF_L3_QUADS)
#define LIDF_AUX_FLOATS 72
#define LIDF_H_NK1 6
#define LIDF_HPASS_QUADS 288
#define LIDF_MAX_L_FUSED 16

enum { LIDF_MODE_FUSED = 0, LIDF_MODE_ROWS = 1, LIDF_MODE_L1ONLY = 2, LIDF_MODE_LINEAR = 3,
       LIDF_MODE_FUSED_H = 4,
       LIDF_MODE_TRAIN = 5,
       LIDF_MODE_ROWS_GATHER = 6,
       LIDF_MODE_PNET_CHAIN = 7,
       LIDF_MODE_IEF16 = 8,
       LIDF_MODE_PNET_BWD = 9,
       LIDF_MODE_CHAIN16 = 10,
       LIDF_MODE_CHAIN16_H = 11 };
#define IEF16_PASS_QUADS 168
#define IEF16_AUX_FLOATS 72

struct NetW {
    const float *w1, *b1, *w2, *b2, *w3, *b3, *w4, *b4, *wenc, *benc;
    int ld1;
    int is_ief;
    int dcore;
};

struct L1Map {
    int n0, c0, n1, c1;
    int D;
    int KQ1;
    int add_bias;
    int nt;
    int nout;
    int transposed;
    int add_u;
    int xcol;
    int L;
    int enter_c0;
    int leave_c0;
};

struct StreamLayout {
    int nets;
    int mode;
    int l1_quads;
    int net_quads;
    int total;
    const struct LidfPackGuardState* guard;
};

#define LIDF_FP_MAX_SEGS 24
#define LIDF_FP_MULTI_SEGS 56
#define LIDF_FP_GROUPS 4

struct LidfPackGuardState {
    unsigned long long hash;
    unsigned long long acc;
    unsigned int ticket;
    int dirty;
    int valid;
    int pad;
};

#define LIDF_PACK_JOBS 13
struct PackJob {
    StreamLayout lay;
    NetW n0, n1;
    L1Map m;
    float* stream;
    float* aux;
};
struct PackJobs {
    PackJob job[LIDF_PACK_JOBS];
    int n;
};


#define PN_P1 1
#define PN_P2 10
#define PN_P3 32
#define PN_P4 68
#define PN_S1_QUADS 16
#define PN_S2_QUADS 112
struct PnetW {
    const float *w_p1, *b_p1, *w_p2, *b_p2, *w_p3, *w_p4, *b_p4;
};
#define PNB_A_QUADS 96
#define PNB_B_QUADS 16
#ifdef __HIPCC__
__device__ __forceinline__ int pn_feature(int s, int half) {
    const int T = s >> 4, r = s & 15;
    return 32 * T + (r & 3) + 8 * (r >> 2) + 4 * half;
}
__device__ __forceinline__ float pn_stream_value(const PnetW& w, int e) {
    int quad = e / 256;
    const int lane = (e % 256) / 4, jj = e & 3;
    const int half = lane >> 5, c32 = lane & 31;
    float v = 0.f;
    if (quad < PN_P1) {
        const int x = 4 * half + jj;
        if (x < 6) v = w.w_p1[c32 * 6 + x];
        else if (x == 6) v = w.b_p1[c32];
    } else if (quad < PN_P1 + PN_P2) {
        quad -= PN_P1;
        const int kq = quad / 2, t = quad % 2, s = 4 * kq + jj, out = 32 * t + c32;
        if (s < 16) v = w.w_p2[out * 32 + pn_feature(s, half)];
        else if (s == 16 && half == 0) v = w.b_p2[out];
    } else if (quad < PN_P1 + PN_P2 + PN_P3) {
        quad -= PN_P1 + PN_P2;
        const int T = quad / 8, kq = quad % 8, s = 4 * kq + jj, out = 32 * T + c32;
        v = w.w_p3[out * 128 + 64 + pn_feature(s, half)];
    } else if (quad < PN_P1 + PN_P2 + PN_P3 + PN_P4) {
        quad -= PN_P1 + PN_P2 + PN_P3;
        const int T = quad / 17, kq = quad % 17, s = 4 * kq + jj, out = 32 * T + c32;
        if (s < 64) v = w.w_p4[out * 128 + pn_feature(s, half)];
        else if (s == 64 && half == 0) v = w.b_p4[out];
    }
    return v;
}
__device__ __forceinline__ float pn_bwd_stream_value(const PnetW& w, int e) {
    const int quad = e / 256;
    const int lane = (e % 256) / 4, jj = e & 3;
    const int half = lane >> 5, c32 = lane & 31;
    float v = 0.f;
    if (quad < 64) {
        const int T = quad / 16, kq = quad % 16;
        v = w.w_p4[pn_feature(4 * kq + jj, half) * 128 + 32 * T + c32];
    } else if (quad < 96) {
        const int q = quad - 64, t = q / 16, kq = q % 16;
        v = w.w_p3[pn_feature(4 * kq + jj, half) * 128 + 64 + 32 * t + c32];
    } else if (quad < 104) {
        const int kq = quad - 96;
        v = w.w_p2[pn_feature(4 * kq + jj, half) * 32 + c32];
    } else if (quad < 108) {
        const int kq = quad - 104;
        if (c32 < 6) v = w.w_p1[pn_feature(4 * kq + jj, half) * 6 + c32];
    }
    return v;
}
#endif

static inline int lidf_l1_quads(int mode, const L1Map& m) {
    if (mode == LIDF_MODE_FUSED) return 24 * ((m.L + 1) / 2) + 8;
    return m.KQ1 * m.nt;
}

static inline StreamLayout lidf_make_layout(int nets, int mode, const L1Map& m) {
    StreamLayout s;
    s.nets = nets;
    s.mode = mode;
    s.l1_quads = lidf_l1_quads(mode, m);
    s.net_quads = s.l1_quads + (mode == LIDF_MODE_L1ONLY || mode == LIDF_MODE_LINEAR ? 0 : LIDF_PASS_QUADS);
    s.total = nets * s.net_quads * 256;
    s.guard = nullptr;
    return s;
}

static inline StreamLayout lidf_make_layout_h(int nets, const L1Map& m) {
    StreamLayout s;
    s.nets = nets;
    s.mode = LIDF_MODE_FUSED_H;
    (void)m;
    s.l1_quads = 0;
    s.net_quads = LIDF_HPASS_QUADS;
    s.total = nets * s.net_quads * 256;
    s.guard = nullptr;
    return s;
}

struct PointsArgs {
    const float* stream;
    const float* aux;
    int nets;
    int l1_quads, net_quads;
    long long n;
    const int* n_dev;
    int npass[2];
    float init[2];
    int sigmoid[2];
    float* out[2];
    int is_offset[2];
    const float* X;
    long long ldx;
    int D, KQ1, has_bias;
    float* out_base;
    const int* pair_ray;
    const int* pair_vox;
    const float* pair_t;
    const float* ray_dir;
    const float* voxpart;
    const float* raypart;
    int part_ld, part_off;
    const float* vox_center;
    int pos_rel, L;
    float r0, rscale, sqrt3, part_size;
    float* pair_pred_pos;
    int* tile_counter;
    int dyn_min_tiles;
    int dyn_chunk;
    int tail_split;
    float* tr_passes[2];
    long long tr_pass_floats;
    float* tr_pre[2];
};

struct LinearArgs {
    const float* stream;
    int kq1;
    const float* X;
    long long ldx, n;
    const int* n_dev;
    int nt_total;
    int D, has_bias;
    const float* addrows;
    const int* addidx;
    int ld_add;
    int relu;
    float* out;
    long long ld_out;
    float* pool;
    const int* poolidx;
// ... 391 lines not shown
```

### implicit_depth_amd/csrc/lidf_dgrad.hip

```cpp
#include "lidf_launch.h"

#define MFMA(a, b, c) __builtin_amdgcn_mfma_f32_32x32x2f32((a), (b), (c), 0, 0, 0)
#define SCHED_FENCE() __builtin_amdgcn_sched_barrier(0)
#define LDQ(rs, voff, soff) \
    __builtin_bit_cast(f32x4, __builtin_amdgcn_raw_buffer_load_b128((rs), (voff), (soff), 0))

#define DG_A_QUADS 32
#define DG_B_QUADS 128
#define DG_QUADS (DG_A_QUADS + DG_B_QUADS)

struct DgradArgs {
    const float* stream;
    const float* dz3;
    const unsigned* m2;
    const unsigned* m1;
    float* dz2;
    float* dz1;
    long long n;
    float slope;
};

__device__ __forceinline__ int dg_feature(int s, int half) {
    const int T = s >> 4, r = s & 15;
    return 32 * T + (r & 3) + 8 * (r >> 2) + 4 * half;
}

__global__ void lidf_pack_dgrad_kernel(const float* __restrict__ w3, const float* __restrict__ w2,
                                       float* __restrict__ stream) {
    const int e = blockIdx.x * blockDim.x + threadIdx.x;
    if (e >= DG_QUADS * 256) return;
    int quad = e / 256;
    const int lane = (e % 256) / 4, jj = e & 3;
    const int half = lane >> 5, c32 = lane & 31;
    float v;
    if (quad < DG_A_QUADS) {
        const int pair = quad / 16, kq = (quad % 16) / 2, t = quad % 2;
        const int k = dg_feature(4 * kq + jj, half);
        v = w3[(size_t)k * LIDF_H2 + 32 * (2 * pair + t) + c32];
    } else {
        quad -= DG_A_QUADS;
        const int pair = quad / 32, kq = (quad % 32) / 2, t = quad % 2;
        const int k = dg_feature(4 * kq + jj, half);
        v = w2[(size_t)k * LIDF_H1 + 32 * (2 * pair + t) + c32];
    }
    stream[e] = v;
}

__device__ __forceinline__ void dg_load_tile(const float* row, int T, f32x4 (&m)[4]) {
#pragma unroll
    for (int g = 0; g < 4; ++g) m[g] = *(const f32x4*)(row + 32 * T + 8 * g);
}
__device__ __forceinline__ float dg_factor(const unsigned* mk, int T, int e, float slope) {
    return (mk[T / 2] & (1u << (31 - (16 * (T & 1) + e)))) ? 1.f : slope;
}
__device__ __forceinline__ void dg_finish_tile(f32x16& acc, const unsigned* mk, float slope,
                                               float* row, int T) {
#pragma unroll
    for (int g = 0; g < 4; ++g) {
        f32x4 o;
#pragma unroll
        for (int i = 0; i < 4; ++i) {
            acc[4 * g + i] *= dg_factor(mk, T, 4 * g + i, slope);
            o[i] = acc[4 * g + i];
        }
        *(f32x4*)(row + 32 * T + 8 * g) = o;
    }
}

template <bool ACC>
__global__ void __launch_bounds__(256, 2) lidf_dgrad_chain_kernel(DgradArgs a) {
    const int lane = threadIdx.x & 63;
    const int wave = threadIdx.x >> 6;
    const int h = lane >> 5;
    const int col = lane & 31;
    const __amdgpu_buffer_rsrc_t srs =
        __builtin_amdgcn_make_buffer_rsrc((void*)a.stream, 0, DG_QUADS * 1024, 0x00020000);
    const int vq = lane * 16;
    const long long ntile = (a.n + 127) / 128;
    const long long per = ntile / gridDim.x, rem = ntile % gridDim.x;
    const long long bx = blockIdx.x;
    const long long tb = bx * per + (bx < rem ? bx : rem);
    const long long te = tb + per + (bx < rem ? 1 : 0);
    if (tb >= te) return;
    const f32x16 zero16 = {0.f, 0.f, 0.f, 0.f, 0.f, 0.f, 0.f, 0.f, 0.f, 0.f, 0.f, 0.f, 0.f, 0.f, 0.f, 0.f};

    f32x4 ring[LIDF_RING];
#pragma unroll
    for (int i = 0; i < LIDF_RING; ++i) ring[i] = LDQ(srs, vq, i * 1024);

    typedef unsigned u32x4 __attribute__((ext_vector_type(4)));
    typedef unsigned u32x2 __attribute__((ext_vector_type(2)));
    f32x4 Bn[2][4];
    u32x2 M2n;
    u32x4 M1n;
    auto request = [&](long long tile) {
        long long p = tile * 128 + wave * 32 + col;
        if (p >= a.n) p = a.n - 1;
        const float* z3 = a.dz3 + (size_t)p * LIDF_H3 + 4 * h;
        M2n = *(const u32x2*)(a.m2 + (size_t)p * 4 + 2 * h);
        M1n = *(const u32x4*)(a.m1 + (size_t)p * 8 + 4 * h);
#pragma unroll
        for (int t = 0; t < 2; ++t) {
#pragma unroll
            for (int g = 0; g < 4; ++g) Bn[t][g] = *(const f32x4*)(z3 + 32 * t + 8 * g);
        }
    };
    request(tb);
    for (long long tile = tb; tile < te; ++tile) {
        if (tile * 128 + wave * 32 >= a.n) break;
        const long long p = tile * 128 + wave * 32 + col;
        const long long pc = p < a.n ? p : a.n - 1;
        const bool valid = p < a.n;
        float* z2 = a.dz2 + (size_t)pc * LIDF_H2 + 4 * h;
        float* z1 = a.dz1 + (size_t)pc * LIDF_H1 + 4 * h;

        f32x16 B3[2];
        unsigned MK2[2], MK1[4];
        MK2[0] = M2n[0]; MK2[1] = M2n[1];
        MK1[0] = M1n[0]; MK1[1] = M1n[1]; MK1[2] = M1n[2]; MK1[3] = M1n[3];
#pragma unroll
        for (int t = 0; t < 2; ++t) {
#pragma unroll
            for (int g = 0; g < 4; ++g) {
#pragma unroll
                for (int i = 0; i < 4; ++i) B3[t][4 * g + i] = Bn[t][g][i];
            }
        }
        SCHED_FENCE();
// ... 79 lines not shown
```

### implicit_depth_amd/csrc/lidf_launch.h

```cpp
#pragma once
#include "lidf_device.h"

extern "C" {

hipError_t lidf_launch_pack_multi(const PackJobs& j, hipStream_t st);
hipError_t lidf_launch_pack(const StreamLayout& lay, const NetW& n0, const NetW& n1, const L1Map& m, float* stream,
                            float* aux, hipStream_t st);
hipError_t lidf_launch_l1only_pair(const PointsArgs& a, const PointsArgs& b, const PointsArgs* c, int cus,
                                   hipStream_t st);
hipError_t lidf_launch_points(int mode, const PointsArgs& a, int grid, hipStream_t st);

hipError_t lidf_launch_pack_h(const StreamLayout& lay, const NetW& n0, const NetW& n1, const L1Map& m, float* stream,
                              float* aux, hipStream_t st);
hipError_t lidf_launch_points_h(const PointsArgs& a, int cus, hipStream_t st);
hipError_t lidf_launch_points_h_list(const PointsArgs& a, int cus, hipStream_t st);

StreamLayout lidf_make_layout_rows_h(int nets, int D, int l1only);
hipError_t lidf_launch_pack_rows_h(const StreamLayout& lay, const NetW& n0, const NetW& n1, const L1Map& m,
                                   float* stream, float* aux, hipStream_t st);
hipError_t lidf_launch_rows_h(const PointsArgs& a, int grid, hipStream_t st);

hipError_t lidf_launch_vox2(const Vox2Args& a, hipStream_t st);
hipError_t lidf_launch_linear(int nt, const LinearArgs& a_in, int grid, hipStream_t st);

// ... 60 lines not shown
                                 int* occ, float* vbound, hipStream_t st);
hipError_t lidf_launch_vox_points(const float* xyz, const int* pt_key, const int* pt_rank, const int* cell_rank,
                                  long long N, const GridSpec& g, int* pid, int* revidx, float* rel, hipStream_t st);
size_t lidf_depth_metrics_ws_bytes(void);
hipError_t lidf_launch_depth_metrics(const float* pred, const float* gt, const void* seg, int seg_dtype, int src_h,
                                     int src_w, int dst_h, int dst_w, float* out, void* ws, hipStream_t st);
hipError_t lidf_launch_miss_block_count(const void* mask, int dtype, long long n, int* block_cnt, hipStream_t st);
hipError_t lidf_launch_miss_count(const void* mask, int dtype, long long n, int* block_cnt, int* block_off, int* sums,
                                  int* n_rays, hipStream_t st);
hipError_t lidf_launch_miss_fill(const void* mask, int dtype, long long n, const int* block_off, const float* intr,
                                 int H, int W, int* ray_bid, int* ray_flat, int* ray_pix, float* ray_dir,
                                 long long* bid64, long long* flat64, long long* pix64, hipStream_t st);
hipError_t lidf_launch_fingerprint(const float* const* ptrs, const long long* floats, int nseg,
                                   unsigned long long salt, LidfPackGuardState* guard, hipStream_t st);
hipError_t lidf_launch_fingerprint_multi(const float* const* ptrs, const long long* floats, const int* grp, int nseg,
                                         const unsigned long long* salts, int ngrp, void* guards, int guard_stride,
                                         hipStream_t st);

size_t lidf_frame_head_blocks(long long npix);
size_t lidf_frame_head_lb_bytes(long long npix);
hipError_t lidf_launch_frame_head(const float* valid_mask, const float* miss_mask, const float* xyz, const float* rgb,
                                  const float* intr, int B, int H, int W, int stride, const GridSpec& g, void* lb,
                                  int* counts, int* valid_bid, int* valid_flat, float* valid_xyz, float* valid_rgb,
                                  int* cell_flag, int* pt_key, int* pt_rank, int* ray_bid, int* ray_flat,
                                  int* ray_pix, float* ray_dir, float* depth, float* depth2, const int* idx_bid,
                                  const int* idx_flat, long long n_list, hipStream_t st);
hipError_t lidf_launch_frame_cells(const int* cell_flag, long long ncell, const GridSpec& g, int* cell_rank, int* occ,
                                   float* vbound, int* vox_bid, float* vox_center, int* counts, int* vox_start,
                                   hipStream_t st);
hipError_t lidf_launch_frame_points(const float* valid_xyz, const float* valid_rgb, const int* pt_key,
                                    const int* pt_rank, const int* cell_rank, const GridSpec& g, long long cap,
                                    const int* counts, int* pid, int* revidx, float* rel, float* pnet_inp,
                                    float* pnet_abs, hipStream_t st);
hipError_t lidf_launch_frame_select(const float* valid_mask, const int* ray_bid, const int* ray_flat, long long hw,
                                    long long R_cap, const int* counts, unsigned char* sel, hipStream_t st);

hipError_t lidf_launch_refine_step(const RefineStepArgs& a, long long R_cap, hipStream_t st);
hipError_t lidf_launch_refine_raystep(const RayStepArgs& a, const CellLookup* cells, hipStream_t st);
hipError_t lidf_launch_refine_prep(const float* pred_pos, const long long* max_pair_id, const int* pair_vox,
                                   long long P, const float* vbound, const int* vox_bid, long long V,
                                   const int* ray_bid, const int* ray_flat, const float* rgb, long long hw,
                                   const float* rayfeat, int ld_rf, int Lv, int L, int pnet_rel, int pos_rel,
                                   long long R, float* pnet_inp, int* pnet_vox, float* inp_embed, int ld_e,
                                   int* end_voxel, const unsigned char* pnet_select, hipStream_t st,
                                   const CellLookup* cells);
hipError_t lidf_launch_refine_prep_dev(const float* pred_pos, const long long* max_pair_id, const int* pair_vox,
                                       long long P, const float* vbound, const int* vox_bid, long long V,
                                       const int* ray_bid, const int* ray_flat, const float* rgb, long long hw,
                                       int pnet_rel, long long R, float* pnet_inp, int* pnet_vox, int* end_voxel,
                                       const unsigned char* pnet_select, const int* dims, const int* row0_dev,
                                       hipStream_t st, const CellLookup* cells);
hipError_t lidf_launch_refine_rows_dev(const float* pred_pos, const int* end_voxel, const float* vbound,
                                       const float* rayfeat, int ld_rf, int Lv, int L, int pos_rel, long long R,
                                       const int* R_dev, float* inp_embed, int ld_e, int pos_only, hipStream_t st);
hipError_t lidf_launch_refine_gather_dev(const float* vox_feat, const int* end_voxel, long long R, const int* R_dev,
                                         float* inp_embed, int ld_e, hipStream_t st);
hipError_t lidf_launch_refine_gather(const float* vox_feat, const int* end_voxel, long long R, float* inp_embed,
                                     int ld_e, hipStream_t st);
hipError_t lidf_launch_refine_finish(const float* pred_pos, const float* off, const float* ray_dir, float r0,
                                     float rs, long long R, float* out, hipStream_t st);
hipError_t lidf_launch_refine_finish_dev(const float* pred_pos, const float* off, const float* ray_dir, float r0,
                                         float rs, long long R, const int* R_dev, float* out, const int* ray_bid,
                                         const int* ray_flat, long long hw, float* depth, hipStream_t st);
hipError_t lidf_launch_refine_train_goff(const float* g, const float* dir, float rs, long long R, const float* pre,
                                         int use_sigmoid, float* goff, hipStream_t st);
hipError_t lidf_launch_refine_train_dcur(const float* g, const float* cur, const int* end_voxel, const float* vbound,
                                         int pos_rel, const float* d_pe, int L, const float* d_inp, long long R,
                                         float* out, hipStream_t st);
hipError_t lidf_launch_add_inplace(float* a, const float* b, long long n, hipStream_t st);
hipError_t lidf_launch_iota(int* p, long long n, hipStream_t st);

hipError_t lidf_launch_wgrad(const float* A, long long lda, int M, const float* B, long long ldb, int N, long long n,
                             float* C, int ldc, float* db, float* g_wgrad_scratch, size_t g_wgrad_scratch_floats,
                             hipStream_t st);
hipError_t lidf_launch_out_act(const float* pre, long long n, int use_sigmoid, float* out, const float* g,
                               float* gpre, hipStream_t st);
hipError_t lidf_launch_l4_backward(const float* goff, const float* h3, const float* w4, float slope, long long n,
                                   float* dz3, float* dw4, float* db4, float* scratch, hipStream_t st);
hipError_t lidf_launch_ief_tail(const float* dz1, const float* off, const float* w1enc, int ld1, const float* wenc,
                                const float* benc, long long n, int s_mode, float* S, float* goff, float* dw1enc,
                                float* dwenc, float* dbenc, float* bacc, float* scratch, hipStream_t st);
hipError_t lidf_launch_ief_first_pass(const float* btot, float* bacc, float init, const float* w1enc, int ld1,
                                      const float* wenc, const float* benc, float* dw1enc, float* dwenc, float* dbenc,
                                      hipStream_t st);
hipError_t lidf_launch_build_rows(const int* pair_ray, const int* pair_vox, const float* pair_t, const float* ray_dir,
                                  const float* vox_center, int pos_rel, const float* vox_feat, const float* rayfeat,
                                  int ld_rf, int L, int Ed, long long P, float* rows, int D, hipStream_t st);
hipError_t lidf_launch_rows_backward(const float* d_rows, int D, int E2, const int* pair_off, const int* pair_vox,
                                     long long R, long long P, int Ed, float* d_vox_feat, float* d_rayfeat, int ld_rf,
                                     hipStream_t st);
hipError_t lidf_launch_rayfeat_backward(const float* d_rayfeat, int ld_rf, const int* ray_pix, const int* ray_bid,
                                        long long R, int half, int B, int H, int W, float* d_feat, float* gimg,
                                        int* aux, hipStream_t st);
hipError_t lidf_launch_pe_rows(const int* pair_ray, const int* pair_vox, const float* pair_t, const float* ray_dir,
                               const float* vox_center, int pos_rel, int L, long long P, float* pe, hipStream_t st,
                               const int* n_dev = nullptr, long long row0 = 0);
hipError_t lidf_launch_seg_sum_ray(const float* S, int F, const int* pair_off, long long R, float* out,
                                   hipStream_t st);
size_t lidf_seg_sum_idx_ws_bytes(long long P, long long V);
hipError_t lidf_launch_seg_sum_idx(const float* S, const int* idx, long long P, long long V, float* out, void* ws,
                                   size_t ws_bytes, hipStream_t st);
size_t lidf_sort_idx_ws_bytes(long long P, long long V);
void lidf_sort_idx_layout(long long P, long long V, size_t* scanned_off, int* nblk, size_t* perm_off);
hipError_t lidf_launch_sort_idx(const int* idx, long long P, const int* n_dev, long long V, void* ws,
                                const int** perm_out, const int** n_perm_out, hipStream_t st);
hipError_t lidf_launch_pair_pos(const float* off, const int* pair_ray, const float* pair_t, const float* ray_dir,
                                long long P, float r0, float rs, float sqrt3, float part, float* out, hipStream_t st,
                                const int* n_dev = nullptr);
hipError_t lidf_launch_ray_select(const float* pos, const long long* id, long long R, long long P, float* pred_pos,
                                  hipStream_t st);
hipError_t lidf_launch_pair_pos_backward(const float* g_pos, const float* g_pred, const long long* id,
                                         const int* pair_ray, const float* ray_dir, long long P, float k,
                                         float* d_off, hipStream_t st);
hipError_t lidf_launch_gather_sel_rows(const float* act, long long P, int npass, const long long* rows, long long R,
                                       const int* pair_vox, const float* pe, int E2, const float* g_pred,
                                       const float* g_extra, const float* ray_dir, float k, float* act_dst, int* pvox,
                                       float* pe_dst, float* g_dst, int* poff, hipStream_t st);
hipError_t lidf_launch_relu_mask(const float* g, const float* src, long long n, float* out, hipStream_t st);
hipError_t lidf_launch_segmax_arg(const float* f, const int* vox, const float* pool, long long N, int F, int* arg,
                                  hipStream_t st);
hipError_t lidf_launch_segmax_backward(const float* dp, const int* arg, const int* vox, const float* pool,
                                       long long N, int F, int accumulate, float* out, hipStream_t st);
hipError_t lidf_launch_seg_sum_rows(const float* S, const int* idx, long long N, int F, float* out, hipStream_t st);
hipError_t lidf_launch_embed_backward(const float* x, const float* g, long long n, int L, float* dx, hipStream_t st);

size_t lidf_roi_align_backward_ws_bytes(long long B, long long H, long long W);
hipError_t lidf_launch_roi_align_backward(const float* d_out, long long ld, const int* ray_pix, const int* ray_bid,
                                          long long R, int B, int Cn, int H, int W, int half, int S, float* d_feat,
                                          void* ws, hipStream_t st);
size_t lidf_seg_sum_idx_any_ws_bytes(long long n, long long V, int F);
hipError_t lidf_launch_seg_sum_idx_any(const float* S, int F, const int* idx, long long n, long long V, float* out,
                                       void* ws, size_t ws_bytes, hipStream_t st);

hipError_t lidf_launch_dgrad_chain(const float* w3, const float* w2, const float* dz3, const unsigned* m2,
                                   const unsigned* m1, long long n, float slope, float* dz2, float* dz1,
                                   int accumulate, float* stream, int cus, hipStream_t st);
size_t lidf_dgrad_stream_bytes(void);
hipError_t lidf_launch_pack_dgrad(const float* w3, const float* w2, float* stream, hipStream_t st);

hipError_t lidf_launch_pack_pointnet(const float* w_p1, const float* b_p1, const float* w_p2, const float* b_p2,
                                     const float* w_p3, const float* w_p4, const float* b_p4, float* stream,
                                     const LidfPackGuardState* guard, hipStream_t st);
size_t lidf_pointnet_chain_stream_bytes(void);
size_t lidf_pointnet_pool_scratch_bytes(long long V);
hipError_t lidf_launch_pointnet_chain(int stage, const float* stream, const float* inp, const int* vox,
                                      const float* gpart, float* pool, float* part, long long V, long long n, int cus,
                                      hipStream_t st);
hipError_t lidf_launch_pointnet_chain_dev(int stage, const float* stream, const float* inp, const int* vox,
                                          const float* gpart, float* pool, long long V_cap, int v_lds,
                                          long long n_cap, const int* n_dev, const int* V_dev, const int* perm,
                                          const int* n_perm, int cus, hipStream_t st);
int lidf_pointnet_lds_max_voxels(void);
size_t lidf_pointnet_sort_bytes(long long n, long long V);
size_t lidf_group_idx_bytes(long long n_cap, long long V);
hipError_t lidf_launch_group_idx(const int* vox, long long n_cap, const int* n_dev, long long V, void* ws,
                                 const int** perm_out, const int** n_perm_out, hipStream_t st);
hipError_t lidf_launch_pointnet_chain_sorted(int stage, const float* stream, const float* inp, const int* vox,
                                             const float* gpart, float* pool, long long V, long long n_cap,
                                             const int* perm, const int* n_perm, int cus, hipStream_t st);

hipError_t lidf_launch_pnet_train_fwd(int stage, const float* stream, const float* inp, const int* vox,
                                      const int* perm, const int* n_perm, const float* gpart, float* inps, int* voxs,
                                      float* f1s, float* f2s, float* f4s, void* pool64, long long V, long long n,
                                      int cus, hipStream_t st);
hipError_t lidf_launch_pnet_unpack(const void* pool64, long long count, float* pool, int* arg, hipStream_t st);
int lidf_pnet_chunk_rows(void);
hipError_t lidf_launch_pnet_tables(const int* scanned, int nblk, long long V, const int* n_perm, int* vstart,
                                   int* first, hipStream_t st);
hipError_t lidf_launch_pnet_bwd_a(const float* stream, const int* voxs, const int* n_perm, const float* dp2,
                                  const int* arg2, const float* f4s, float* dz4s, float* df2s, long long n, int cus,
                                  hipStream_t st);
hipError_t lidf_launch_pnet_bwd_b(const float* stream, const int* voxs, const int* perm, const int* n_perm,
                                  const float* df2s, const float* dp1, const int* arg1, const float* f2s,
                                  const float* f1s, float* dz2s, float* dz1s, float* d_inp, long long n, int cus,
                                  hipStream_t st);
hipError_t lidf_launch_pnet_dw4(const float* dp2, const int* arg2, const float* f4s, long long V, float* dW4,
// ... 44 lines not shown
```

### implicit_depth_amd/csrc/lidf_points.hip

```cpp
#include "lidf_launch.h"

#define MFMA(a, b, c) __builtin_amdgcn_mfma_f32_32x32x2f32((a), (b), (c), 0, 0, 0)
#define SCHED_FENCE() __builtin_amdgcn_sched_barrier(0)

#ifdef LIDF_PROFILE
#define PROF_DECL long long prof_t = clock64(); long long prof_acc[8] = {0, 0, 0, 0, 0, 0, 0, 0}; const long long prof_c0 = prof_t, prof_w0 = wall_clock64();
#define PROF(i) { long long t_ = clock64(); prof_acc[i] += t_ - prof_t; prof_t = t_; }
#define PROF_DUMP if (blockIdx.x == 0 && threadIdx.x == 0 && a.out_base) { for (int i_ = 0; i_ < 8; ++i_) ((long long*)a.out_base)[i_] = prof_acc[i_]; } \
    if ((threadIdx.x & 63) == 0 && a.out_base) { long long* o_ = (long long*)a.out_base + 16 + 4 * (blockIdx.x * 4 + (threadIdx.x >> 6)); o_[0] = prof_w0; o_[1] = wall_clock64(); o_[2] = clock64() - prof_c0; }
#else
#define PROF_DECL
#define PROF(i)
#define PROF_DUMP
#endif

typedef unsigned int u32x4 __attribute__((ext_vector_type(4)));
#define LDQ(rs, voff, soff) \
    __builtin_bit_cast(f32x4, __builtin_amdgcn_raw_buffer_load_b128((rs), (voff), (soff), 0))

__device__ __forceinline__ int k_to_feature(int s, int half) {
    int T = s >> 4, r = s & 15;
    return 32 * T + (r & 3) + 8 * (r >> 2) + 4 * half;
}

// ... 122 lines not shown
        const int tile = 4 * quad + r;
        return (g == 0 && tile < T2) ? n.b2[16 * tile + j] : 0.f;
    }
    quad -= NB2;
    const int blk_len = 1 + 4 * T2;
    if (quad < (T1 / 4) * blk_len) {
        const int blk = quad / blk_len, in = quad % blk_len;
        if (in == 0) return (g == 0 && n.is_ief) ? ief_u(n, 16 * (4 * blk + r) + j) : 0.f;
        const int T = 4 * blk + (in - 1) / T2, To = (in - 1) % T2;
        return n.w2[(size_t)(16 * To + j) * (64 * G) + 16 * T + 4 * g + r];
    }
    quad -= (T1 / 4) * blk_len;
    if (quad < NB3) {
        const int tile = 4 * quad + r;
        return (g == 0 && tile < T3) ? n.b3[16 * tile + j] : 0.f;
    }
    quad -= NB3;
    if (quad < T2 * T3) {
        const int T = quad / T3, To = quad % T3;
        return n.w3[(size_t)(16 * To + j) * (32 * G) + 16 * T + 4 * g + r];
    }
    return 0.f;
}

__device__ float chain16h_pieces(float w0, float w1, int lo) {
    typedef _Float16 h2p __attribute__((ext_vector_type(2)));
    const _Float16 h0 = (_Float16)w0, h1 = (_Float16)w1;
    const h2p pk = {lo ? (_Float16)(w0 - (float)h0) : h0, lo ? (_Float16)(w1 - (float)h1) : h1};
    return __builtin_bit_cast(float, pk);
}
__device__ float chain16h_stream_value(const NetW& n, const L1Map& m, int e) {
    const int G = m.nt, T1 = 4 * G, T2 = 2 * G, T3 = G;
    const int KP = ((m.n0 + 15) / 16 + 1) / 2;
    int quad = e / 256;
    const int lane = (e % 256) / 4, c = e & 3;
    const int j = lane & 15, g = lane >> 4;
    const int f0 = 16 * (c >> 1) + 4 * g + 2 * (c & 1);
    if (quad < KP * 2 * T1) {
        const int kp = quad / (2 * T1), To = (quad % (2 * T1)) / 2, x = 32 * kp + f0;
        const float* w = n.w1 + (size_t)(16 * To + j) * n.ld1 + m.c0;
        return chain16h_pieces(x < m.n0 ? w[x] : 0.f, x + 1 < m.n0 ? w[x + 1] : 0.f, quad & 1);
    }
    quad -= KP * 2 * T1;
    const int NB2 = (T2 + 3) / 4, NB3 = (T3 + 3) / 4;
    if (quad < NB2) {
        const int tile = 4 * quad + c;
        return (g == 0 && tile < T2) ? n.b2[16 * tile + j] : 0.f;
    }
    quad -= NB2;
    const int blk_len = 1 + 4 * T2;
    if (quad < (T1 / 4) * blk_len) {
        const int blk = quad / blk_len, in = quad % blk_len;
        if (in == 0) return (g == 0 && n.is_ief) ? ief_u(n, 16 * (4 * blk + c) + j) : 0.f;
        const int pair = (in - 1) / (2 * T2), To = ((in - 1) % (2 * T2)) / 2;
        const float* w = n.w2 + (size_t)(16 * To + j) * (64 * G) + 16 * (4 * blk + 2 * pair) + f0;
        return chain16h_pieces(w[0], w[1], (in - 1) & 1);
    }
    quad -= (T1 / 4) * blk_len;
    if (quad < NB3) {
        const int tile = 4 * quad + c;
        return (g == 0 && tile < T3) ? n.b3[16 * tile + j] : 0.f;
    }
    quad -= NB3;
    if (quad < T2 * T3) {
        const int pair = quad / (2 * T3), To = (quad % (2 * T3)) / 2;
        const float* w = n.w3 + (size_t)(16 * To + j) * (32 * G) + 32 * pair + f0;
        return chain16h_pieces(w[0], w[1], quad & 1);
    }
    return 0.f;
}

__device__ __forceinline__ void pack_body(const StreamLayout& lay, const NetW& net0, const NetW& net1,
                                          const L1Map& m, float* stream, float* aux) {
    if (lay.guard && lay.guard->dirty == 0) return;
    int e = blockIdx.x * blockDim.x + threadIdx.x;
    if (lay.mode == LIDF_MODE_PNET_CHAIN) {
        const PnetW w = {net0.w1, net0.b1, net0.w2, net0.b2, net0.w3, net0.b3, net0.w4};
        if (e < lay.total) stream[e] = pn_stream_value(w, e);
        return;
    }
    if (lay.mode == LIDF_MODE_PNET_BWD) {
        const PnetW w = {net0.w1, net0.b1, net0.w2, net0.b2, net0.w3, net0.b3, net0.w4};
        if (e < lay.total) stream[e] = pn_bwd_stream_value(w, e);
        return;
    }
    if (lay.mode == LIDF_MODE_IEF16) {
        if (e < lay.total) stream[e] = ief16_stream_value(net0, m, e);
        if (e < IEF16_AUX_FLOATS)
            aux[e] = e < 64 ? net0.w4[e] : (e == 64 ? net0.b4[0] : 0.f);
        return;
    }
    if (lay.mode == LIDF_MODE_CHAIN16 || lay.mode == LIDF_MODE_CHAIN16_H) {
        const int gf = 16 * m.nt;
        if (e < lay.total)
            stream[e] = lay.mode == LIDF_MODE_CHAIN16 ? chain16_stream_value(net0, m, e) : chain16h_stream_value(net0, m, e);
        if (e < gf + 8) aux[e] = e < gf ? net0.w4[e] : (e == gf ? net0.b4[0] : 0.f);
        return;
    }
    if (e < lay.total) stream[e] = stream_value(lay, net0, net1, m, e);
    if (lay.mode != LIDF_MODE_L1ONLY && lay.mode != LIDF_MODE_LINEAR && e < lay.nets * LIDF_AUX_FLOATS) {
        int sec = e / LIDF_AUX_FLOATS, i = e % LIDF_AUX_FLOATS;
        const NetW& n = sec ? net1 : net0;
        float v = 0.f;
        if (i < 64) {
            int half = i / 32, s = i % 32;
            v = n.w4[k_to_feature(s, half)];
        } else if (i == 64) {
            v = n.b4[0];
        }
        aux[e] = v;
    }
}

__global__ void lidf_pack_kernel(StreamLayout lay, NetW net0, NetW net1, L1Map m, float* stream,
                                 float* aux) {
    pack_body(lay, net0, net1, m, stream, aux);
}

__global__ void lidf_pack_multi_kernel(PackJobs j) {
    const PackJob& k = j.job[blockIdx.y];
    pack_body(k.lay, k.n0, k.n1, k.m, k.stream, k.aux);
}

extern "C" hipError_t lidf_launch_pack_multi(const PackJobs& j, hipStream_t st) {
    if (j.n <= 0) return hipSuccess;
    int blocks = 1;
    for (int i = 0; i < j.n; ++i) {
        const StreamLayout& lay = j.job[i].lay;
        const int total = lay.total > lay.nets * LIDF_AUX_FLOATS ? lay.total : lay.nets * LIDF_AUX_FLOATS;
        const int b = (total + 255) / 256;
        blocks = b > blocks ? b : blocks;
    }
    hipLaunchKernelGGL(lidf_pack_multi_kernel, dim3(blocks, j.n), dim3(256), 0, st, j);
    return hipGetLastError();
}

extern "C" hipError_t lidf_launch_pack(const StreamLayout& lay, const NetW& n0, const NetW& n1,
                                       const L1Map& m, float* stream, float* aux,
                                       hipStream_t st) {
    int total = lay.total > lay.nets * LIDF_AUX_FLOATS ? lay.total : lay.nets * LIDF_AUX_FLOATS;
    int blocks = (total + 255) / 256;
    hipLaunchKernelGGL(lidf_pack_kernel, dim3(blocks), dim3(256), 0, st, lay, n0, n1, m, stream,
                       aux);
    return hipGetLastError();
}

template <int LO, int HI>
__device__ __forceinline__ void lrelu_part(f32x16& v) {
#pragma unroll
    for (int i = LO; i < HI; i += 2) {
        f32x2 x = {v[i], v[i + 1]};
        f32x2 t;
        const f32x2 slope = {0.02f, 0.02f};
        asm("v_pk_mul_f32 %0, %1, %2" : "=v"(t) : "v"(x), "v"(slope));
        float r0, r1;
        asm("v_max_f32 %0, %1, %2" : "=v"(r0) : "v"(x[0]), "v"(t[0]));
        asm("v_max_f32 %0, %1, %2" : "=v"(r1) : "v"(x[1]), "v"(t[1]));
        v[i] = r0;
        v[i + 1] = r1;
    }
}

__device__ __forceinline__ float out_act(float y, int use_sigmoid) {
    if (use_sigmoid) return 1.f / (1.f + expf(-y));
    return fmaxf(fminf(y, y * 0.01f + 0.99f), y * 0.01f);
}
// ... 1023 lines not shown
```

### implicit_depth_amd/csrc/lidf_train.hip

```cpp
#include "lidf_launch.h"
#include <stdlib.h>

#define MFMA(a, b, c) __builtin_amdgcn_mfma_f32_32x32x2f32((a), (b), (c), 0, 0, 0)

struct WgradArgs {
    const float* A; long long lda; int M;
    const float* B; long long ldb; int N;
    long long n;
    float* C; int ldc;
    float* db;
    int mtiles, ntiles, splits;
    long long rows_per_split;
};

__global__ void __launch_bounds__(256) lidf_wgrad_kernel(WgradArgs a) {
    const int lane = threadIdx.x & 63, wave = threadIdx.x >> 6;
    const int h = lane >> 5, c = lane & 31;
    long long id = (long long)blockIdx.x * 4 + wave;
    if (id >= (long long)a.mtiles * a.ntiles * a.splits) return;
    const int mt = (int)(id % a.mtiles); id /= a.mtiles;
    const int nt = (int)(id % a.ntiles); id /= a.ntiles;
    const long long r0 = id * a.rows_per_split;
    long long r1 = r0 + a.rows_per_split;
    if (r1 > a.n) r1 = a.n;
// ... 576 lines not shown
                for (int i = 0; i < 4; ++i) {
                    A[i] = fmaf(v[j][i], o[j], A[i]);
                    B[i] += v[j][i];
                }
            }
        }
    }
    if (!w1enc) return;
    red[wave][0][lane] = A;
    red[wave][1][lane] = B;
    __syncthreads();
    if (threadIdx.x < 128) {
        const int which = threadIdx.x >> 6, l = threadIdx.x & 63;
        f32x4w s = red[0][which][l];
#pragma unroll
        for (int k = 1; k < 4; ++k) s += red[k][which][l];
        *(f32x4w*)(part + (size_t)blockIdx.x * 512 + 256 * which + 4 * l) = s;
    }
}

__global__ void __launch_bounds__(256) lidf_colsum_reduce_kernel(const float* __restrict__ part, int G,
                                                                 int ncol, float* __restrict__ out) {
    __shared__ float red[16][16];
    const int k = threadIdx.x >> 4, cl = threadIdx.x & 15, c = blockIdx.x * 16 + cl;
    float s = 0.f;
    if (c < ncol) {
        int g = k;
        for (; g + 112 < G; g += 128) {
            float x[8];
#pragma unroll
            for (int j = 0; j < 8; ++j) x[j] = part[(size_t)(g + 16 * j) * ncol + c];
#pragma unroll
            for (int j = 0; j < 8; ++j) s += x[j];
        }
        for (; g < G; g += 16) s += part[(size_t)g * ncol + c];
    }
    red[k][cl] = s;
    __syncthreads();
    if (k == 0 && c < ncol) {
        float t = red[0][cl];
#pragma unroll
        for (int j = 1; j < 16; ++j) t += red[j][cl];
        out[c] = t;
    }
}

__global__ void lidf_l4_finish_kernel(const float* __restrict__ sums, float* __restrict__ dw4,
                                      float* __restrict__ db4) {
    const int c = threadIdx.x;
    if (c < 64) dw4[c] += sums[c];
    if (c == 64) db4[0] += sums[64];
}
__global__ void __launch_bounds__(256) lidf_l4_reduce_finish_kernel(const float* __restrict__ part, int G,
                                                                    float* __restrict__ dw4,
                                                                    float* __restrict__ db4) {
    __shared__ float red[16][16];
    const int k = threadIdx.x >> 4, cl = threadIdx.x & 15, c = blockIdx.x * 16 + cl;
    float s = 0.f;
    if (c < 65) {
        int g = k;
        for (; g + 112 < G; g += 128) {
            float x[8];
#pragma unroll
            for (int j = 0; j < 8; ++j) x[j] = part[(size_t)(g + 16 * j) * 65 + c];
#pragma unroll
            for (int j = 0; j < 8; ++j) s += x[j];
        }
        for (; g < G; g += 16) s += part[(size_t)g * 65 + c];
    }
    red[k][cl] = s;
    __syncthreads();
    if (k == 0 && c < 65) {
        float t = red[0][cl];
#pragma unroll
        for (int j = 1; j < 16; ++j) t += red[j][cl];
        if (c < 64) dw4[c] += t;
        else db4[0] += t;
    }
}

__global__ void __launch_bounds__(256) lidf_ief_finish_kernel(
    const float* __restrict__ sums, const float* __restrict__ w1enc, int ld1,
    const float* __restrict__ wenc, const float* __restrict__ benc, float* __restrict__ dw1enc,
    float* __restrict__ dwenc, float* __restrict__ dbenc, float* __restrict__ bacc,
    const float* __restrict__ btot, float init) {
    __shared__ float sA[256], sB[256];
    const int c = threadIdx.x;
    float A, B;
    if (btot) {
        B = btot[c] - bacc[c];
        A = init * B;
    } else {
        A = sums[c];
        B = sums[256 + c];
        if (bacc) bacc[c] += B;
    }
    sA[c] = A;
    sB[c] = B;
#pragma unroll
    for (int j = 0; j < 16; ++j) dw1enc[(size_t)c * ld1 + j] += fmaf(wenc[j], A, benc[j] * B);
    __syncthreads();
    __shared__ float sp[8][32];
    {
        const int j = c & 15, which = (c >> 4) & 1, piece = c >> 5;
        const float* v = which ? sB : sA;
        float t = 0.f;
#pragma unroll 8
        for (int i = 32 * piece; i < 32 * piece + 32; ++i) t = fmaf(w1enc[(size_t)i * ld1 + j], v[i], t);
        sp[piece][c & 31] = t;
    }
    __syncthreads();
    if (c < 32) {
        float t = sp[0][c];
#pragma unroll
        for (int k = 1; k < 8; ++k) t += sp[k][c];
        if (c < 16) dwenc[c] += t;
        else dbenc[c - 16] += t;
    }
}

static inline long long narrow_rows_per_wg(long long n, int* G) {
    long long g = (n + 255) / 256;
    if (g > 1024) g = 1024;
    if (g < 1) g = 1;
    const long long rows = ((n + g - 1) / g + 15) / 16 * 16;
    *G = (int)((n + rows - 1) / rows);
    return rows;
}

extern "C" hipError_t lidf_launch_l4_backward(const float* goff, const float* h3, const float* w4,
                                              float slope, long long n, float* dz3, float* dw4,
                                              float* db4, float* scratch, hipStream_t st) {
    if (n <= 0) return hipSuccess;
    int G;
    const long long rows = narrow_rows_per_wg(n, &G);
    float* sums = scratch + (size_t)G * 65;
    hipLaunchKernelGGL(lidf_l4_backward_kernel, dim3(G), dim3(256), 0, st, goff, h3, w4, slope, n,
                       rows, dz3, scratch);
    (void)sums;
    hipLaunchKernelGGL(lidf_l4_reduce_finish_kernel, dim3(5), dim3(256), 0, st, scratch, G, dw4, db4);
    return hipGetLastError();
}

extern "C" hipError_t lidf_launch_ief_tail(const float* dz1, const float* off, const float* w1enc,
                                           int ld1, const float* wenc, const float* benc,
                                           long long n, int s_mode, float* S, float* goff,
                                           float* dw1enc, float* dwenc, float* dbenc,
                                           float* bacc, float* scratch, hipStream_t st) {
    if (n <= 0 || (!w1enc && s_mode == 0)) return hipSuccess;
    int G;
    const long long rows = narrow_rows_per_wg(n, &G);
    float* sums = scratch + (size_t)G * 512;
    hipLaunchKernelGGL(lidf_ief_tail_kernel, dim3(G), dim3(256), 0, st, dz1, off, w1enc, ld1, wenc,
                       n, rows, s_mode, S, goff, scratch);
    if (w1enc) {
        hipLaunchKernelGGL(lidf_colsum_reduce_kernel, dim3(32), dim3(256), 0, st, scratch, G, 512, sums);
        hipLaunchKernelGGL(lidf_ief_finish_kernel, dim3(1), dim3(256), 0, st, sums, w1enc, ld1, wenc,
                           benc, dw1enc, dwenc, dbenc, bacc, (const float*)nullptr, 0.f);
    }
    return hipGetLastError();
}

extern "C" hipError_t lidf_launch_ief_first_pass(const float* btot, float* bacc, float init,
                                                 const float* w1enc, int ld1, const float* wenc,
                                                 const float* benc, float* dw1enc, float* dwenc,
                                                 float* dbenc, hipStream_t st) {
    hipLaunchKernelGGL(lidf_ief_finish_kernel, dim3(1), dim3(256), 0, st, (const float*)nullptr, w1enc,
                       ld1, wenc, benc, dw1enc, dwenc, dbenc, bacc, btot, init);
    return hipGetLastError();
}

__global__ void __launch_bounds__(256) lidf_build_rows_kernel(
    const int* __restrict__ pair_ray, const int* __restrict__ pair_vox, const float* __restrict__ pair_t,
    const float* __restrict__ ray_dir, const float* __restrict__ vox_center, int pos_rel,
    const float* __restrict__ vox_feat, const float* __restrict__ rayfeat, int ld_rf, int L, int Ed,
    long long P, float* __restrict__ rows, int D) {
    const int lane = threadIdx.x & 63;
    const long long p = (long long)blockIdx.x * 4 + (threadIdx.x >> 6);
    if (p >= P) return;
    const int r = pair_ray[p], v = pair_vox[p];
    const float te = pair_t[2 * p], tl = pair_t[2 * p + 1];
    const float d[3] = {ray_dir[3 * (size_t)r], ray_dir[3 * (size_t)r + 1], ray_dir[3 * (size_t)r + 2]};
    float c[3] = {0.f, 0.f, 0.f};
    if (pos_rel) {
        c[0] = vox_center[3 * (size_t)v];
        c[1] = vox_center[3 * (size_t)v + 1];
        c[2] = vox_center[3 * (size_t)v + 2];
    }
    const int E = 3 + 6 * L;
    float* o = rows + (size_t)p * D;
    for (int j = lane; j < D; j += 64) {
        float val;
        if (j < 128) {
            val = vox_feat[(size_t)v * 128 + j];
        } else if (j < 256) {
            val = rayfeat[(size_t)r * ld_rf + (j - 128)];
        } else if (j < 256 + 2 * E) {
            const int k = (j - 256) % E;
            const float t = j - 256 < E ? te : tl;
            const int i = k < 3 ? k : (k - 3) % 3;
            const float x = __fmul_rn(d[i], t) - c[i];
            if (k < 3) {
                val = x;
            } else {
                const int oct = (k - 3) / 6;
                const float a = x * (float)(1 << oct);
                val = ((k - 3) % 6) < 3 ? sinf(a) : cosf(a);
            }
        } else {
            val = rayfeat[(size_t)r * ld_rf + 128 + (j - 256 - 2 * E)];
        }
        o[j] = val;
    }
}

__global__ void __launch_bounds__(256) lidf_rows_ray_backward_kernel(
    const float* __restrict__ d_rows, int D, int E2, const int* __restrict__ pair_off, long long R,
    int Ed, float* __restrict__ d_rayfeat, int ld_rf) {
    const int lane = threadIdx.x & 63;
    const long long r = (long long)blockIdx.x * 4 + (threadIdx.x >> 6);
    if (r >= R) return;
    const int beg = pair_off[r], end = pair_off[r + 1];
    for (int j = lane; j < 128 + Ed; j += 64) {
        const int colr = j < 128 ? 128 + j : 256 + E2 + (j - 128);
        float acc = 0.f;
        for (int p = beg; p < end; ++p) acc += d_rows[(size_t)p * D + colr];
        d_rayfeat[(size_t)r * ld_rf + j] = acc;
    }
}

__global__ void __launch_bounds__(256) lidf_rows_vox_backward_kernel(
    const float* __restrict__ d_rows, int D, const int* __restrict__ pair_vox, long long P,
    float* __restrict__ d_vox_feat) {
    const long long i = (long long)blockIdx.x * 256 + threadIdx.x;
    if (i >= P * 128) return;
    const long long p = i >> 7;
    const int j = (int)(i & 127);
    const float g = d_rows[(size_t)p * D + j];
    if (g != 0.f) atomicAdd(d_vox_feat + (size_t)pair_vox[p] * 128 + j, g);
}

__global__ void lidf_rayfeat_count_kernel(const int* __restrict__ ray_pix, const int* __restrict__ ray_bid,
                                          long long R, int H, int W, int* __restrict__ pix_rays) {
    const long long r = (long long)blockIdx.x * blockDim.x + threadIdx.x;
    if (r >= R) return;
    atomicAdd(pix_rays + ((size_t)ray_bid[r] * H + ray_pix[2 * r + 1]) * W + ray_pix[2 * r], 1);
}

__device__ __forceinline__ void roi_tap(float x, int LIM, int& lo, int& hi, float& l, bool& ok) {
    ok = !(x < -1.0f || x > (float)LIM);
    if (x <= 0.f) x = 0.f;
// ... 113 lines not shown
            if (alone) *dst = g;
            else atomicAdd(dst, g);
            continue;
        }
        const int c = cb >> 2, ph = (cb >> 1) & 1, pw = cb & 1;
        const float gs = g / (float)max(gh * gw, 1);
        float* img = d_feat + ((size_t)bid * 32 + c) * H * W;
        for (int iy = 0; iy < gh; ++iy) {
            float y = rsh + (float)ph * bin_h + ((float)iy + .5f) * bin_h / (float)gh;
            for (int ix = 0; ix < gw; ++ix) {
                float x = rsw + (float)pw * bin_w + ((float)ix + .5f) * bin_w / (float)gw;
                float yy = y;
                if (yy < -1.0f || yy > (float)H || x < -1.0f || x > (float)W) continue;
                if (yy <= 0.f) yy = 0.f;
                if (x <= 0.f) x = 0.f;
                int y_low = (int)yy, x_low = (int)x, y_high, x_high;
                if (y_low >= H - 1) { y_high = y_low = H - 1; yy = (float)y_low; } else { y_high = y_low + 1; }
                if (x_low >= W - 1) { x_high = x_low = W - 1; x = (float)x_low; } else { x_high = x_low + 1; }
                const float ly = yy - (float)y_low, lx = x - (float)x_low, hy = 1.f - ly, hx = 1.f - lx;
                if (hy * hx != 0.f) atomicAdd(img + y_low * W + x_low, gs * hy * hx);
                if (hy * lx != 0.f) atomicAdd(img + y_low * W + x_high, gs * hy * lx);
                if (ly * hx != 0.f) atomicAdd(img + y_high * W + x_low, gs * ly * hx);
                if (ly * lx != 0.f) atomicAdd(img + y_high * W + x_high, gs * ly * lx);
            }
        }
    }
}

extern "C" hipError_t lidf_launch_build_rows(const int* pair_ray, const int* pair_vox,
                                             const float* pair_t, const float* ray_dir,
                                             const float* vox_center, int pos_rel,
                                             const float* vox_feat, const float* rayfeat, int ld_rf,
                                             int L, int Ed, long long P, float* rows, int D,
                                             hipStream_t st) {
    if (P <= 0) return hipSuccess;
    hipLaunchKernelGGL(lidf_build_rows_kernel, dim3((unsigned)((P + 3) / 4)), dim3(256), 0, st,
                       pair_ray, pair_vox, pair_t, ray_dir, vox_center, pos_rel, vox_feat, rayfeat,
                       ld_rf, L, Ed, P, rows, D);
    return hipGetLastError();
}

extern "C" hipError_t lidf_launch_rows_backward(const float* d_rows, int D, int E2,
                                                const int* pair_off, const int* pair_vox,
                                                long long R, long long P, int Ed, float* d_vox_feat,
                                                float* d_rayfeat, int ld_rf, hipStream_t st) {
    if (d_rayfeat && R > 0)
        hipLaunchKernelGGL(lidf_rows_ray_backward_kernel, dim3((unsigned)((R + 3) / 4)), dim3(256), 0,
                           st, d_rows, D, E2, pair_off, R, Ed, d_rayfeat, ld_rf);
    if (d_vox_feat && P > 0)
        hipLaunchKernelGGL(lidf_rows_vox_backward_kernel, dim3((unsigned)((P * 128 + 255) / 256)),
                           dim3(256), 0, st, d_rows, D, pair_vox, P, d_vox_feat);
    return hipGetLastError();
}

__global__ void __launch_bounds__(256) lidf_rayfeat_gather_kernel(const float* __restrict__ gimg,
                                                                  int B, int H, int W, int half, int lo,
                                                                  float* __restrict__ d_feat) {
    const long long i = (long long)blockIdx.x * 256 + threadIdx.x;
    const long long total = (long long)B * 32 * H * W;
    if (i >= total) return;
    const int x = (int)(i % W), y = (int)((i / W) % H);
    const long long bc = i / ((long long)W * H);
    const long long b = bc / 32;
    const int c = (int)(bc % 32);
    float acc = 0.f;
#pragma unroll
    for (int ph = 0; ph < 2; ++ph) {
        const int ya = ph ? y - half + 1 : y + 1, yb = ph ? y : y + half;
#pragma unroll
        for (int pw = 0; pw < 2; ++pw) {
            const int xa = pw ? x - half + 1 : x + 1, xb = pw ? x : x + half;
            const float* g = gimg + ((size_t)(b * 128 + c * 4 + ph * 2 + pw) * H) * W;
            for (int yy = max(ya, lo); yy <= min(yb, H - 1 - lo); ++yy)
                for (int xx = max(xa, lo); xx <= min(xb, W - 1 - lo); ++xx) acc += g[(size_t)yy * W + xx];
        }
    }
    d_feat[i] += acc / (float)(half * half);
}

extern "C" hipError_t lidf_launch_rayfeat_backward(const float* d_rayfeat, int ld_rf,
                                                   const int* ray_pix, const int* ray_bid,
                                                   long long R, int half, int B, int H, int W,
                                                   float* d_feat, float* gimg, int* aux,
                                                   hipStream_t st) {
    if (R <= 0) return hipSuccess;
    if (half <= 0) gimg = nullptr;
    const int tx_n = (W + 15) / 16, ty_n = (H + 15) / 16;
    if (!gimg || half > 16 || W < 2 * half + 1 || H < 2 * half + 1 || W - 16 * (tx_n - 1) < half ||
        H - 16 * (ty_n - 1) < half)
        aux = nullptr;
    if (gimg) {
        hipError_t e = hipMemsetAsync(gimg, 0, (size_t)B * 128 * H * W * 4, st);
        if (e != hipSuccess) return e;
    }
    if (aux) {
        hipError_t e = hipMemsetAsync(aux, 0, (size_t)B * H * W * 4, st);
        if (e != hipSuccess) return e;
        hipLaunchKernelGGL(lidf_rayfeat_count_kernel, dim3((unsigned)((R + 255) / 256)), dim3(256), 0, st,
                           ray_pix, ray_bid, R, H, W, aux);
    }
    hipLaunchKernelGGL(lidf_rayfeat_backward_kernel, dim3((unsigned)((R + 63) / 64)), dim3(256), 0,
                       st, d_rayfeat, ld_rf, ray_pix, ray_bid, R, half, H, W, d_feat, gimg, aux,
                       aux ? 1 : 0);
    if (gimg) {
        const long long total = (long long)B * 32 * H * W;
        hipLaunchKernelGGL(lidf_rayfeat_gather_kernel, dim3((unsigned)((total + 255) / 256)),
                           dim3(256), 0, st, gimg, B, H, W, half, aux ? half : 0, d_feat);
    }
    if (aux) {
        const int side = ty_n > 2 ? (tx_n > 1 ? 2 : 1) * (ty_n - 2) : 0;
        const int tiles = (ty_n > 1 ? 2 * tx_n : tx_n) + side;
        const int PW = 18 + 2 * half;
        hipLaunchKernelGGL(lidf_rayfeat_backward_ring_kernel, dim3(tiles, B * 32), dim3(256),
                           (size_t)PW * PW * 4, st, gimg, half, H, W, d_feat);
    }
    return hipGetLastError();
}

__global__ void __launch_bounds__(256) lidf_pe_rows_kernel(
    const int* __restrict__ pair_ray, const int* __restrict__ pair_vox, const float* __restrict__ pair_t,
    const float* __restrict__ ray_dir, const float* __restrict__ vox_center, int pos_rel, int L,
    long long P, float* __restrict__ pe, const int* __restrict__ n_dev, long long row0) {
    if (n_dev) {
        const long long m = (long long)*n_dev - row0;
        P = m < P ? (m > 0 ? m : 0) : P;
    }
    if ((long long)blockIdx.x * 32 >= P) return;
    __shared__ __attribute__((aligned(16))) float s_rows[32 * 2 * (3 + 6 * 16)];
    const int E = 3 + 6 * L, W = 2 * E;
    const long long p0 = (long long)blockIdx.x * 32;
    const long long p = p0 + (threadIdx.x >> 3);
    const int q = threadIdx.x & 7;
    if (p < P && q < 6) {
        const int end = q >= 3 ? 1 : 0, c = q - 3 * end;
        float x = __fmul_rn(ray_dir[3 * (size_t)pair_ray[p] + c], pair_t[2 * p + end]);
        if (pos_rel) x -= vox_center[3 * (size_t)pair_vox[p] + c];
        float* row = s_rows + (threadIdx.x >> 3) * W + end * E;
        row[c] = x;
        const Rev r = to_rev(x);
        for (int o = 0; o < L; ++o) {
            float sn, cs;
            rev_sincos(r, (float)(1 << o), sn, cs);
            row[3 + 6 * o + c] = sn;
            row[6 + 6 * o + c] = cs;
        }
    }
    __syncthreads();
    const long long rows = P - p0 < 32 ? P - p0 : 32;
    const int total = (int)rows * W;
    float* dst = pe + (size_t)p0 * W;
    for (int i = 4 * threadIdx.x; i + 3 < total; i += 1024) *(f32x4*)(dst + i) = *(const f32x4*)(s_rows + i);
    if (threadIdx.x < (total & 3)) dst[(total & ~3) + threadIdx.x] = s_rows[(total & ~3) + threadIdx.x];
}

__global__ void __launch_bounds__(256) lidf_seg_sum_ray_kernel(const float* __restrict__ S, int F,
                                                               const int* __restrict__ pair_off,
                                                               long long R, float* __restrict__ out) {
    const int lane = threadIdx.x & 63;
    const long long r = (long long)blockIdx.x * 4 + (threadIdx.x >> 6);
    if (r >= R) return;
    const int beg = pair_off[r], end = pair_off[r + 1];
    for (int j = lane * 4; j < F; j += 256) {
        f32x4 acc = {0.f, 0.f, 0.f, 0.f};
        for (int p = beg; p < end; ++p) {
            const f32x4 v = *(const f32x4*)(S + (size_t)p * F + j);
#pragma unroll
            for (int i = 0; i < 4; ++i) acc[i] += v[i];
        }
        *(f32x4*)(out + (size_t)r * F + j) = acc;
    }
}

__global__ void __launch_bounds__(256) lidf_seg_sum_idx_kernel(const float* __restrict__ S,
                                                               const int* __restrict__ idx,
                                                               long long P, float* __restrict__ out) {
    const int lane = threadIdx.x & 63;
    const long long p0 = ((long long)blockIdx.x * 4 + (threadIdx.x >> 6)) * 64;
    if (p0 >= P) return;
    const long long p1 = p0 + 64 < P ? p0 + 64 : P;
    f32x4 acc = {0.f, 0.f, 0.f, 0.f};
// ... 496 lines not shown
```

Measured before the change: 388.7.

## Batch weight-pack and zeroing launches into fewer multi-segment kernels

```diff
diff --git a/implicit_depth_amd/csrc/lidf_api.hip b/implicit_depth_amd/csrc/lidf_api.hip
--- a/implicit_depth_amd/csrc/lidf_api.hip
+++ b/implicit_depth_amd/csrc/lidf_api.hip
@@ -44,6 +44,14 @@
     PackJob& k = tl_jobs->job[tl_jobs->n++];
     k.lay = guarded(lay); k.n0 = n0; k.n1 = n1; k.m = m; k.stream = stream; k.aux = aux;
     return hipSuccess;
+}
+static hipError_t pack_dgrad_stream(const float* w3, const float* w2, float* stream, hipStream_t st) {
+    if (!tl_jobs) return lidf_launch_pack_dgrad(w3, w2, stream, st);
+    StreamLayout lay = {};
+    lay.nets = 1; lay.mode = LIDF_MODE_DGRAD; lay.total = DG_QUADS * 256;
+    NetW n = {};
+    n.w3 = w3; n.w2 = w2;
+    return pack_stream(lay, n, n, L1Map{}, stream, nullptr, st);
 }
 struct JobScope {
     PackJobs jobs;
@@ -65,12 +73,13 @@
     return LIDF_OK;
 }
 
-static hipError_t zero_decoder_grads(const LidfDecoderGrads* g, int ld1, int is_ief, hipStream_t st) {
-    float* const p[10] = {g->w1, g->b1, g->w2, g->b2, g->w3, g->b3, g->w4, g->b4,
-                          is_ief ? g->wenc : nullptr, is_ief ? g->benc : nullptr};
-    const long long c[10] = {(long long)LIDF_H1 * ld1, LIDF_H1, (long long)LIDF_H2 * LIDF_H1, LIDF_H2,
-                             (long long)LIDF_H3 * LIDF_H2, LIDF_H3, LIDF_H3, 1, 16, 16};
-    return lidf_launch_zero_segments(p, c, 10, st);
+static hipError_t zero_decoder_grads(const LidfDecoderGrads* g, int ld1, int is_ief, hipStream_t st,
+                                     float* x0 = nullptr, long long n0 = 0, float* x1 = nullptr, long long n1 = 0) {
+    float* const p[12] = {g->w1, g->b1, g->w2, g->b2, g->w3, g->b3, g->w4, g->b4,
+                          is_ief ? g->wenc : nullptr, is_ief ? g->benc : nullptr, x0, x1};
+    const long long c[12] = {(long long)LIDF_H1 * ld1, LIDF_H1, (long long)LIDF_H2 * LIDF_H1, LIDF_H2,
+                             (long long)LIDF_H3 * LIDF_H2, LIDF_H3, LIDF_H3, 1, 16, 16, n0, n1};
+    return lidf_launch_zero_segments(p, c, 12, st);
 }
 
 static int check_decoder(const LidfDecoder* d) {
@@ -2647,14 +2656,17 @@
 }
 
 struct TrainWs {
-    size_t stream, dz1, dz2, dz3, S, goff, wg, chain, small, total;
+    size_t stream, dgs, inp, dz1, dz2, dz3, S, goff, wg, chain, small, total;
 };
+static inline int input_grad_slots(int d) { return ((d + 31) / 32 + 7) / 8; }
 static TrainWs train_ws(int64_t n, int d) {
     TrainWs w;
     const size_t N = (size_t)(n > 0 ? n : 1);
     size_t o = 0;
     const int kmax = d > 256 ? d : 256;
     w.stream = o; o += linex_stream_bytes(kmax);
+    w.dgs = o;    o += align_up(lidf_dgrad_stream_bytes(), 256);
+    w.inp = o;    o += (size_t)input_grad_slots(d) * linex_stream_bytes(LIDF_H1);
     w.dz1 = o;    o += align_up(N * LIDF_H1 * 4, 256);
     w.dz2 = o;    o += align_up(N * LIDF_H2 * 4, 256);
     w.dz3 = o;    o += align_up(N * LIDF_H3 * 4, 256);
@@ -2702,7 +2714,7 @@
                                  const TrainWs& w, int cus, hipStream_t st, float** S_out) {
     const int npass = dec->is_ief ? dec->n_iter : 1;
     const int ld1 = d + (dec->is_ief ? 16 : 0);
-    float* sbuf = (float*)(ws + w.stream);
+    float* sbuf = (float*)(ws + w.dgs);
     float* dz1 = (float*)(ws + w.dz1);
     float* dz2 = (float*)(ws + w.dz2);
     float* dz3 = (float*)(ws + w.dz3);
@@ -2711,9 +2723,7 @@
     const float* pre = act + (size_t)npass * n * ACT_ROW_FLOATS;
     float* S = (float*)(ws + w.S);
     float* small = (float*)(ws + w.small);
-    CHECK_HIP(hipMemsetAsync(small, 0, 512 * 4, st));
     CHECK_HIP(lidf_launch_out_act(pre, n, dec->use_sigmoid, nullptr, g_out, goff, st));
-    CHECK_HIP(lidf_launch_pack_dgrad(dec->w3, dec->w2, sbuf, st));
     if (npass == 1) S = dz1;
     for (int k = npass - 1; k >= 0; --k) {
         const float* h1 = act_h1(act, n, k);
@@ -2749,7 +2759,7 @@
 
 static int decoder_input_grad(const float* S, const LidfDecoder* dec, const float* S2, const LidfDecoder* dec2,
                               int64_t n, int32_t d, float* d_inp, int64_t ld_dinp, float* sbuf, int cus,
-                              hipStream_t st) {
+                              hipStream_t st, int pack_mode) {
     LinEx L = {};
     L.n = n; L.transposed = 1; L.mask_slope = 0.02f;
     const int ld1 = d + (dec->is_ief ? 16 : 0);
@@ -2771,7 +2781,8 @@
         }
         L.out = d_inp + c0; L.ld_out = ld_dinp; L.accumulate = 0;
         int rc;
-        if ((rc = run_linex(L, sbuf, cus, st))) return rc;
+        float* slot = (float*)((char*)sbuf + (size_t)(c0 / (32 * per)) * linex_stream_bytes(S2 ? 2 * LIDF_H1 : LIDF_H1));
+        if ((rc = run_linex(L, slot, cus, st, pack_mode))) return rc;
     }
     return LIDF_OK;
 }
@@ -2787,22 +2798,31 @@
     if ((rc = check_decoder_grads(dec, grads))) return rc;
     if (d_inp && ld_dinp < d) return LIDF_ERR_BAD_ARG;
     hipStream_t st = (hipStream_t)stream;
-    CHECK_HIP(zero_decoder_grads(grads, d + (dec->is_ief ? 16 : 0), dec->is_ief, st));
+    const TrainWs w = train_ws(n, d);
+    char* ws = (char*)workspace;
+    const bool run = n > 0 && inp && act && g_out && workspace && workspace_bytes >= w.total;
+    CHECK_HIP(zero_decoder_grads(grads, d + (dec->is_ief ? 16 : 0), dec->is_ief, st,
+                                 run ? (float*)(ws + w.small) : nullptr, 512));
     if (n == 0) return LIDF_OK;
     if (!inp || !act || !g_out) return LIDF_ERR_BAD_ARG;
-    const TrainWs w = train_ws(n, d);
     if (!workspace || workspace_bytes < w.total) return LIDF_ERR_WORKSPACE;
-    char* ws = (char*)workspace;
     int cus;
     if ((rc = cu_count(&cus))) return rc;
     float* S = nullptr;
+    {
+        JobScope js;
+        CHECK_HIP(pack_dgrad_stream(dec->w3, dec->w2, (float*)(ws + w.dgs), st));
+        if (d_inp && (rc = decoder_input_grad(S, dec, nullptr, nullptr, n, d, d_inp, ld_dinp, (float*)(ws + w.inp), cus, st, 1)))
+            return rc;
+        CHECK_HIP(flush_jobs(js.jobs, st));
+    }
     if ((rc = decoder_backward_core(inp, n, d, ld_inp, dec, act, g_out, grads, ws, w, cus, st, &S))) return rc;
-    if (d_inp) return decoder_input_grad(S, dec, nullptr, nullptr, n, d, d_inp, ld_dinp, (float*)(ws + w.stream), cus, st);
+    if (d_inp) return decoder_input_grad(S, dec, nullptr, nullptr, n, d, d_inp, ld_dinp, (float*)(ws + w.inp), cus, st, 2);
     return LIDF_OK;
 }
 
 LIDF_API size_t lidf_decoder_pair_workspace_bytes(int64_t n, int32_t d) {
-    return 2 * align_up(train_ws(n, d).total, 256) + linex_stream_bytes(2 * LIDF_H1);
+    return 2 * align_up(train_ws(n, d).total, 256) + (size_t)input_grad_slots(d) * linex_stream_bytes(2 * LIDF_H1);
 }
 LIDF_API size_t lidf_decoder_pair_workspace_offset(int64_t n, int32_t d, int32_t which) {
     return (size_t)(which ? 1 : 0) * align_up(train_ws(n, d).total, 256);
@@ -2821,20 +2841,33 @@
     if ((rc = check_decoder_grads(prob, grads_prob)) || (rc = check_decoder_grads(off, grads_off))) return rc;
     if (d_inp && ld_dinp < d) return LIDF_ERR_BAD_ARG;
     hipStream_t st = (hipStream_t)stream;
-    CHECK_HIP(zero_decoder_grads(grads_prob, d + (prob->is_ief ? 16 : 0), prob->is_ief, st));
-    CHECK_HIP(zero_decoder_grads(grads_off, d + (off->is_ief ? 16 : 0), off->is_ief, st));
+    const TrainWs w = train_ws(n, d);
+    const size_t one = align_up(w.total, 256);
+    char* ws = (char*)workspace;
+    const bool run = n > 0 && inp && act_prob && act_off && g_prob && g_off && workspace &&
+                     workspace_bytes >= lidf_decoder_pair_workspace_bytes(n, d);
+    CHECK_HIP(zero_decoder_grads(grads_prob, d + (prob->is_ief ? 16 : 0), prob->is_ief, st,
+                                 run ? (float*)(ws + w.small) : nullptr, 512));
+    CHECK_HIP(zero_decoder_grads(grads_off, d + (off->is_ief ? 16 : 0), off->is_ief, st,
+                                 run ? (float*)(ws + one + w.small) : nullptr, 512));
     if (n == 0) return LIDF_OK;
     if (!inp || !act_prob || !act_off || !g_prob || !g_off) return LIDF_ERR_BAD_ARG;
-    const TrainWs w = train_ws(n, d);
-    const size_t one = align_up(w.total, 256);
     if (!workspace || workspace_bytes < lidf_decoder_pair_workspace_bytes(n, d)) return LIDF_ERR_WORKSPACE;
-    char* ws = (char*)workspace;
     int cus;
     if ((rc = cu_count(&cus))) return rc;
     float *Sp = nullptr, *So = nullptr;
+    {
+        JobScope js;
+        CHECK_HIP(pack_dgrad_stream(prob->w3, prob->w2, (float*)(ws + w.dgs), st));
+        CHECK_HIP(pack_dgrad_stream(off->w3, off->w2, (float*)(ws + one + w.dgs), st));
+        if (d_inp && (rc = decoder_input_grad(nullptr, prob, (const float*)ws, off, n, d, d_inp, ld_dinp,
+                                              (float*)(ws + 2 * one), cus, st, 1)))
+            return rc;
+        CHECK_HIP(flush_jobs(js.jobs, st));
+    }
     if ((rc = decoder_backward_core(inp, n, d, ld_inp, prob, act_prob, g_prob, grads_prob, ws, w, cus, st, &Sp))) return rc;
     if ((rc = decoder_backward_core(inp, n, d, ld_inp, off, act_off, g_off, grads_off, ws + one, w, cus, st, &So))) return rc;
-    if (d_inp) return decoder_input_grad(Sp, prob, So, off, n, d, d_inp, ld_dinp, (float*)(ws + 2 * one), cus, st);
+    if (d_inp) return decoder_input_grad(Sp, prob, So, off, n, d, d_inp, ld_dinp, (float*)(ws + 2 * one), cus, st, 2);
     return LIDF_OK;
 }
 
@@ -2881,16 +2914,17 @@
                                               lidf_stream_t stream) {
     if (n_rays < 0 || batch <= 0 || height <= 0 || width <= 0 || !d_feat_grid) return LIDF_ERR_BAD_ARG;
     hipStream_t st = (hipStream_t)stream;
-    CHECK_HIP(hipMemsetAsync(d_feat_grid, 0, (size_t)batch * 32 * height * width * 4, st));
-    if (n_rays == 0) return LIDF_OK;
-    if (!d_rayfeat || !ray_pix || !ray_bid) return LIDF_ERR_BAD_ARG;
+    if (n_rays == 0 || !d_rayfeat || !ray_pix || !ray_bid) {
+        CHECK_HIP(zero_words(d_feat_grid, (size_t)batch * 32 * height * width, nullptr, 0, st));
+        return n_rays == 0 ? LIDF_OK : LIDF_ERR_BAD_ARG;
+    }
     const size_t need = (size_t)batch * 128 * height * width * 4;
     const size_t need2 = need + (size_t)batch * height * width * 4;
     float* gimg = (workspace && workspace_bytes >= need) ? (float*)workspace : nullptr;
     int* pix_rays = (workspace && workspace_bytes >= need2) ? (int*)((char*)workspace + need) : nullptr;
     CHECK_HIP(lidf_launch_rayfeat_backward(d_rayfeat, 128 + 3 + 6 * multires_views, ray_pix, ray_bid,
                                            n_rays, roi_inp_bbox / 2, batch, height, width, d_feat_grid,
-                                           gimg, pix_rays, st));
+                                           gimg, pix_rays, st, 1));
     return LIDF_OK;
 }
 
@@ -2916,13 +2950,18 @@
 }
 
 struct QTrainWs {
-    size_t stream, dz1, dz2, dz3, S, goff, dvox, dray, wg, seg, seg_bytes, chain, small, total;
+    size_t stream, dgs, s_dvox, s_dpe, s_dray0, s_dray1, dz1, dz2, dz3, S, goff, dvox, dray, wg, seg, seg_bytes, chain, small, total;
 };
 static QTrainWs qtrain_ws(int64_t P, int64_t R, int64_t V) {
     QTrainWs w;
     const size_t N = (size_t)(P > 0 ? P : 1);
     size_t o = 0;
     w.stream = o; o += linex_stream_bytes(256);
+    w.dgs = o;    o += align_up(lidf_dgrad_stream_bytes(), 256);
+    w.s_dvox = o; o += linex_stream_bytes(256);
+    w.s_dpe = o;  o += linex_stream_bytes(256);
+    w.s_dray0 = o; o += linex_stream_bytes(256);
+    w.s_dray1 = o; o += linex_stream_bytes(256);
     w.dz1 = o;    o += align_up(N * LIDF_H1 * 4, 256);
     w.dz2 = o;    o += align_up(N * LIDF_H2 * 4, 256);
     w.dz3 = o;    o += align_up(N * LIDF_H3 * 4, 256);
@@ -3033,7 +3072,11 @@
     hipStream_t st = (hipStream_t)stream;
     char* ws = (char*)workspace;
     const QueryPlan p = query_plan(L, Lv, LIDF_PRECISION_F32);
-    if ((rc = pack_query_weights(q->dec, offset_dec, p, ws, st))) return rc;
+    {
+        JobScope js;
+        if ((rc = pack_query_weights(q->dec, offset_dec, p, ws, st))) return rc;
+        CHECK_HIP(flush_jobs(js.jobs, st));
+    }
     int cus;
     if ((rc = cu_count(&cus))) return rc;
     CHECK_HIP(lidf_launch_l1only_pair(
@@ -3087,7 +3130,11 @@
     if (!workspace || workspace_bytes < w.total) return LIDF_ERR_WORKSPACE;
     char* ws = (char*)workspace;
     const QueryPlan p = query_plan(L, Lv, LIDF_PRECISION_F32);
-    if ((rc = pack_query_weights(q->dec, offset_dec, p, ws, st))) return rc;
+    {
+        JobScope js;
+        if ((rc = pack_query_weights(q->dec, offset_dec, p, ws, st))) return rc;
+        CHECK_HIP(flush_jobs(js.jobs, st));
+    }
     int cus;
     if ((rc = cu_count(&cus))) return rc;
     CHECK_HIP(lidf_launch_l1only_pair(
@@ -3131,6 +3178,7 @@
     float *s_dvox, *s_dpe;
     int pack_mode;
     const float* s_dgrad;
+    bool small_clear;
     bool goff_ready;
     const float* l1rows;
     int l1_ld, l1_cols, l1_c0;
@@ -3147,7 +3195,6 @@
     const int E2 = o.E2, Ed = 3 + 6 * q->multires_views;
     const int D = 256 + E2 + Ed, ld1 = D + (dec->is_ief ? 16 : 0);
     const int npass = dec->is_ief ? dec->n_iter : 1;
-    float* sbuf = (float*)(ws + w.stream);
     float* dz1 = (float*)(ws + w.dz1);
     float* dz2 = (float*)(ws + w.dz2);
     float* dz3 = (float*)(ws + w.dz3);
@@ -3157,13 +3204,34 @@
     float* dvox = (float*)(ws + w.dvox);
     float* dray = (float*)(ws + w.dray);
     float* small = (float*)(ws + w.small);
-    CHECK_HIP(hipMemsetAsync(small, 0, 512 * 4, st));
+    const auto input_grads = [&](int mode) -> int {
+        LinEx L = {};
+        L.transposed = 1; L.ldw = ld1; L.k = LIDF_H1; L.ldx = LIDF_H1; L.accumulate = accumulate_inputs ? 1 : 0;
+        if (d_vox_feat) {
+            L.w = dec->w1; L.nout = 128; L.X = dvox; L.n = V; L.out = d_vox_feat; L.ld_out = 128;
+            if ((rc = run_linex(L, o.s_dvox ? o.s_dvox : (float*)(ws + w.s_dvox), cus, st, mode))) return rc;
+        }
+        if (o.d_pe) {
+            L.w = dec->w1 + 256; L.nout = E2; L.X = S; L.n = P; L.out = o.d_pe; L.ld_out = E2; L.accumulate = 0;
+            if ((rc = run_linex(L, o.s_dpe ? o.s_dpe : (float*)(ws + w.s_dpe), cus, st, mode))) return rc;
+            L.accumulate = accumulate_inputs ? 1 : 0;
+        }
+        if (d_rayfeat && !o.S_keep) {
+            L.w = dec->w1 + 128; L.nout = 128; L.X = dray; L.n = R; L.out = d_rayfeat; L.ld_out = 128 + Ed;
+            if ((rc = run_linex(L, (float*)(ws + w.s_dray0), cus, st, mode))) return rc;
+            L.w = dec->w1 + 256 + E2; L.nout = Ed; L.out = d_rayfeat + 128;
+            if ((rc = run_linex(L, (float*)(ws + w.s_dray1), cus, st, mode))) return rc;
+        }
+        return LIDF_OK;
+    };
+    const float* dgs = o.s_dgrad ? o.s_dgrad : (const float*)(ws + w.dgs);
+    if (!o.s_dgrad || !o.s_dvox) {
+        JobScope js;
+        if (!o.s_dgrad) CHECK_HIP(pack_dgrad_stream(dec->w3, dec->w2, (float*)(ws + w.dgs), st));
+        if (!o.s_dvox && (rc = input_grads(1))) return rc;
+        CHECK_HIP(flush_jobs(js.jobs, st));
+    }
     if (!o.goff_ready) CHECK_HIP(lidf_launch_out_act(pre, P, dec->use_sigmoid, nullptr, g_out, goff, st));
-    const float* dgs = o.s_dgrad;
-    if (!dgs) {
-        CHECK_HIP(lidf_launch_pack_dgrad(dec->w3, dec->w2, sbuf, st));
-        dgs = sbuf;
-    }
     for (int k = npass - 1; k >= 0; --k) {
         const float* h1 = passes + (size_t)k * qact_pass(P);
         const float* h2 = h1 + (size_t)P * LIDF_H1;
@@ -3196,7 +3264,7 @@
     if (short_first)
         CHECK_HIP(lidf_launch_ief_first_pass(small + 256, small, dec->init_offset, dec->w1 + D, ld1,
                                              dec->wenc, dec->benc, grads->w1 + D, grads->wenc,
-                                             grads->benc, st));
+                                             grads->benc, st, o.small_clear ? 1 : 0));
     if (o.ss_perm)
         CHECK_HIP(lidf_launch_pnet_gather_segsum(S, o.ss_perm, o.ss_row0, o.ss_vstart, o.ss_first, V, o.ss_n,
                                                  o.ss_partial, dvox, st));
@@ -3209,24 +3277,7 @@
         CHECK_HIP(lidf_launch_wgrad(dray, LIDF_H1, LIDF_H1, q->rayfeat, 128 + Ed, 128, R, grads->w1 + 128, ld1, nullptr, wgs, WG_SCRATCH_FLOATS, st));
         CHECK_HIP(lidf_launch_wgrad(dray, LIDF_H1, LIDF_H1, q->rayfeat + 128, 128 + Ed, Ed, R, grads->w1 + 256 + E2, ld1, nullptr, wgs, WG_SCRATCH_FLOATS, st));
     }
-    LinEx L = {};
-    L.transposed = 1; L.ldw = ld1; L.k = LIDF_H1; L.ldx = LIDF_H1; L.accumulate = accumulate_inputs ? 1 : 0;
-    if (d_vox_feat) {
-        L.w = dec->w1; L.nout = 128; L.X = dvox; L.n = V; L.out = d_vox_feat; L.ld_out = 128;
-        if ((rc = run_linex(L, o.s_dvox ? o.s_dvox : sbuf, cus, st, o.s_dvox ? o.pack_mode : 0))) return rc;
-    }
-    if (o.d_pe) {
-        L.w = dec->w1 + 256; L.nout = E2; L.X = S; L.n = P; L.out = o.d_pe; L.ld_out = E2; L.accumulate = 0;
-        if ((rc = run_linex(L, o.s_dpe ? o.s_dpe : sbuf, cus, st, o.s_dpe ? o.pack_mode : 0))) return rc;
-        L.accumulate = accumulate_inputs ? 1 : 0;
-    }
-    if (d_rayfeat && !o.S_keep) {
-        L.w = dec->w1 + 128; L.nout = 128; L.X = dray; L.n = R; L.out = d_rayfeat; L.ld_out = 128 + Ed;
-        if ((rc = run_linex(L, sbuf, cus, st))) return rc;
-        L.w = dec->w1 + 256 + E2; L.nout = Ed; L.out = d_rayfeat + 128;
-        if ((rc = run_linex(L, sbuf, cus, st))) return rc;
-    }
-    return LIDF_OK;
+    return input_grads(o.s_dvox ? o.pack_mode : 2);
 }
 
 LIDF_API int lidf_query_decoder_backward_f32(const LidfQueryTrainArgs* q, const float* act,
@@ -3246,14 +3297,17 @@
     const int E2 = 2 * (3 + 6 * q->multires), Ed = 3 + 6 * q->multires_views;
     const int D = 256 + E2 + Ed, ld1 = D + (dec->is_ief ? 16 : 0);
     const int npass = dec->is_ief ? dec->n_iter : 1;
-    CHECK_HIP(zero_decoder_grads(grads, ld1, dec->is_ief, st));
-    if (!accumulate_inputs) {
-        if (d_vox_feat && V > 0) CHECK_HIP(hipMemsetAsync(d_vox_feat, 0, (size_t)V * 128 * 4, st));
-        if (d_rayfeat && R > 0) CHECK_HIP(hipMemsetAsync(d_rayfeat, 0, (size_t)R * (128 + Ed) * 4, st));
+    const QTrainWs w = qtrain_ws(P, R, V);
+    const bool run = P > 0 && act && g_out && workspace && workspace_bytes >= w.total;
+    if (!run) {
+        const bool z = !accumulate_inputs;
+        CHECK_HIP(zero_decoder_grads(grads, ld1, dec->is_ief, st, z && V > 0 ? d_vox_feat : nullptr, V * 128,
+                                     z && R > 0 ? d_rayfeat : nullptr, R * (128 + Ed)));
+    } else {
+        CHECK_HIP(zero_decoder_grads(grads, ld1, dec->is_ief, st, (float*)((char*)workspace + w.small), 512));
     }
     if (P == 0) return LIDF_OK;
     if (!act || !g_out) return LIDF_ERR_BAD_ARG;
-    const QTrainWs w = qtrain_ws(P, R, V);
     if (!workspace || workspace_bytes < w.total) return LIDF_ERR_WORKSPACE;
     int cus;
     if ((rc = cu_count(&cus))) return rc;
@@ -3306,14 +3360,17 @@
     const int E2 = 2 * (3 + 6 * q->multires), Ed = 3 + 6 * q->multires_views;
     const int D = 256 + E2 + Ed, ld1 = D + (dec->is_ief ? 16 : 0);
     const int npass = dec->is_ief ? dec->n_iter : 1;
-    CHECK_HIP(zero_decoder_grads(grads, ld1, dec->is_ief, st));
-    if (!accumulate_inputs) {
-        if (d_vox_feat && V > 0) CHECK_HIP(hipMemsetAsync(d_vox_feat, 0, (size_t)V * 128 * 4, st));
-        if (d_rayfeat && R > 0) CHECK_HIP(hipMemsetAsync(d_rayfeat, 0, (size_t)R * (128 + Ed) * 4, st));
+    const QRowsWs l = qrows_ws(R, V, E2, npass);
+    const bool run = P > 0 && R > 0 && act && rows && ray_dir && workspace && workspace_bytes >= l.total;
+    if (!run) {
+        const bool z = !accumulate_inputs;
+        CHECK_HIP(zero_decoder_grads(grads, ld1, dec->is_ief, st, z && V > 0 ? d_vox_feat : nullptr, V * 128,
+                                     z && R > 0 ? d_rayfeat : nullptr, R * (128 + Ed)));
+    } else {
+        CHECK_HIP(zero_decoder_grads(grads, ld1, dec->is_ief, st, (float*)((char*)workspace + l.inner + l.w.small), 512));
     }
     if (P == 0 || R == 0) return LIDF_OK;
     if (!act || !rows || !ray_dir) return LIDF_ERR_BAD_ARG;
-    const QRowsWs l = qrows_ws(R, V, E2, npass);
     if (!workspace || workspace_bytes < l.total) return LIDF_ERR_WORKSPACE;
     int cus;
     if ((rc = cu_count(&cus))) return rc;
diff --git a/implicit_depth_amd/csrc/lidf_api_refine_train.inc b/implicit_depth_amd/csrc/lidf_api_refine_train.inc
--- a/implicit_depth_amd/csrc/lidf_api_refine_train.inc
+++ b/implicit_depth_amd/csrc/lidf_api_refine_train.inc
@@ -195,10 +195,10 @@
                                    (float*)(act + l.s_ray), act + l.s_chain, cus, st, 1);
         if (!rc)
             rc = rt_pack_transposed(dec, E, Ed, (float*)(act + l.s_dvox), (float*)(act + l.s_dpe), cus, st);
+        if (!rc && pack_dgrad_stream(dec->w3, dec->w2, (float*)(act + l.s_dgrad), st) != hipSuccess) rc = LIDF_ERR_HIP;
         if (!rc && flush_jobs(js.jobs, st) != hipSuccess) rc = LIDF_ERR_HIP;
         if (rc) return rc;
     }
-    CHECK_HIP(lidf_launch_pack_dgrad(dec->w3, dec->w2, (float*)(act + l.s_dgrad), st));
     CHECK_HIP(lidf_launch_iota(ray_idx, R, st));
     if ((rc = qdec_forward_impl(&t, E, nullptr, nullptr, raypart, nullptr, nullptr, nullptr, (float*)(act + l.s_ray),
                                 nullptr, cus, st, 2, 2)))
@@ -274,7 +274,13 @@
     const int D = refine_D(q->multires, q->multires_views), ld1 = D + (dec->is_ief ? 16 : 0);
     const int npass = dec->is_ief ? dec->n_iter : 1;
     hipStream_t st = (hipStream_t)stream;
-    CHECK_HIP(zero_decoder_grads(gd, ld1, dec->is_ief, st));
+    float* small0 = nullptr;
+    if (R > 0 && g_pos && act_v && q->workspace) {
+        const RtWs w0 = rt_ws(R, Nv, V, E);
+        if (q->workspace_bytes >= w0.total && act_bytes >= rt_lay(R, Nv, V, E, npass, T).total)
+            small0 = (float*)((char*)q->workspace + w0.qd + w0.qw.small);
+    }
+    CHECK_HIP(zero_decoder_grads(gd, ld1, dec->is_ief, st, small0, 512));
     {
         float* const zp[12] = {gp->w_p1, gp->b_p1, gp->w_p2, gp->b_p2, gp->w_v1, gp->b_v1, gp->w_p3, gp->b_p3,
                                gp->w_p4, gp->b_p4, gp->w_v2, gp->b_v2};
@@ -323,6 +329,7 @@
         o.s_dvox = (float*)(act + l.s_dvox); o.s_dpe = (float*)(act + l.s_dpe); o.pack_mode = 2;
         o.s_dgrad = (const float*)(act + l.s_dgrad);
         o.goff_ready = true;
+        o.small_clear = true;
         if (chain) {
             const PnetActC pc = pnetc_act(n, V);
             size_t sc_off, perm_off;
@@ -357,13 +364,18 @@
     }
     (void)wgs;
     if (d_rayfeat) {
-        float* sbuf = (float*)(ws + w.qd + w.qw.stream);
+        float* s0 = (float*)(ws + w.qd + w.qw.s_dray0);
+        float* s1 = (float*)(ws + w.qd + w.qw.s_dray1);
         LinEx L = {};
         L.transposed = 1; L.ldw = ld1; L.k = LIDF_H1; L.ldx = LIDF_H1; L.X = ssum; L.n = R;
-        L.w = dec->w1 + 128; L.nout = 128; L.out = d_rayfeat; L.ld_out = 128 + Ed;
-        if ((rc = run_linex(L, sbuf, cus, st))) return rc;
-        L.w = dec->w1 + 256 + E; L.nout = Ed; L.out = d_rayfeat + 128;
-        if ((rc = run_linex(L, sbuf, cus, st))) return rc;
+        for (int mode = 1; mode <= 2; ++mode) {
+            JobScope js;
+            L.w = dec->w1 + 128; L.nout = 128; L.out = d_rayfeat; L.ld_out = 128 + Ed;
+            if ((rc = run_linex(L, s0, cus, st, mode))) return rc;
+            L.w = dec->w1 + 256 + E; L.nout = Ed; L.out = d_rayfeat + 128;
+            if ((rc = run_linex(L, s1, cus, st, mode))) return rc;
+            if (mode == 1) CHECK_HIP(flush_jobs(js.jobs, st));
+        }
     }
     return LIDF_OK;
 }
diff --git a/implicit_depth_amd/csrc/lidf_device.h b/implicit_depth_amd/csrc/lidf_device.h
--- a/implicit_depth_amd/csrc/lidf_device.h
+++ b/implicit_depth_amd/csrc/lidf_device.h
@@ -37,7 +37,8 @@
        LIDF_MODE_IEF16 = 8,
        LIDF_MODE_PNET_BWD = 9,
        LIDF_MODE_CHAIN16 = 10,
-       LIDF_MODE_CHAIN16_H = 11 };
+       LIDF_MODE_CHAIN16_H = 11,
+       LIDF_MODE_DGRAD = 12 };
 #define IEF16_PASS_QUADS 168
 #define IEF16_AUX_FLOATS 72
 
@@ -160,6 +161,26 @@
         if (c32 < 6) v = w.w_p1[pn_feature(4 * kq + jj, half) * 6 + c32];
     }
     return v;
+}
+#endif
+
+#define DG_A_QUADS 32
+#define DG_B_QUADS 128
+#define DG_QUADS (DG_A_QUADS + DG_B_QUADS)
+#ifdef __HIPCC__
+__device__ __forceinline__ float dg_stream_value(const float* __restrict__ w3, const float* __restrict__ w2, int e) {
+    int quad = e / 256;
+    const int lane = (e % 256) / 4, jj = e & 3;
+    const int half = lane >> 5, c32 = lane & 31;
+    if (quad < DG_A_QUADS) {
+        const int pair = quad / 16, kq = (quad % 16) / 2, t = quad % 2;
+        const int k = pn_feature(4 * kq + jj, half);
+        return w3[(size_t)k * LIDF_H2 + 32 * (2 * pair + t) + c32];
+    }
+    quad -= DG_A_QUADS;
+    const int pair = quad / 32, kq = (quad % 32) / 2, t = quad % 2;
+    const int k = pn_feature(4 * kq + jj, half);
+    return w2[(size_t)k * LIDF_H1 + 32 * (2 * pair + t) + c32];
 }
 #endif
 
diff --git a/implicit_depth_amd/csrc/lidf_dgrad.hip b/implicit_depth_amd/csrc/lidf_dgrad.hip
--- a/implicit_depth_amd/csrc/lidf_dgrad.hip
+++ b/implicit_depth_amd/csrc/lidf_dgrad.hip
@@ -5,9 +5,6 @@
 #define LDQ(rs, voff, soff) \
     __builtin_bit_cast(f32x4, __builtin_amdgcn_raw_buffer_load_b128((rs), (voff), (soff), 0))
 
-#define DG_A_QUADS 32
-#define DG_B_QUADS 128
-#define DG_QUADS (DG_A_QUADS + DG_B_QUADS)
 
 struct DgradArgs {
     const float* stream;
@@ -20,30 +17,11 @@
     float slope;
 };
 
-__device__ __forceinline__ int dg_feature(int s, int half) {
-    const int T = s >> 4, r = s & 15;
-    return 32 * T + (r & 3) + 8 * (r >> 2) + 4 * half;
-}
-
 __global__ void lidf_pack_dgrad_kernel(const float* __restrict__ w3, const float* __restrict__ w2,
                                        float* __restrict__ stream) {
     const int e = blockIdx.x * blockDim.x + threadIdx.x;
     if (e >= DG_QUADS * 256) return;
-    int quad = e / 256;
-    const int lane = (e % 256) / 4, jj = e & 3;
-    const int half = lane >> 5, c32 = lane & 31;
-    float v;
-    if (quad < DG_A_QUADS) {
-        const int pair = quad / 16, kq = (quad % 16) / 2, t = quad % 2;
-        const int k = dg_feature(4 * kq + jj, half);
-        v = w3[(size_t)k * LIDF_H2 + 32 * (2 * pair + t) + c32];
-    } else {
-        quad -= DG_A_QUADS;
-        const int pair = quad / 32, kq = (quad % 32) / 2, t = quad % 2;
-        const int k = dg_feature(4 * kq + jj, half);
-        v = w2[(size_t)k * LIDF_H1 + 32 * (2 * pair + t) + c32];
-    }
-    stream[e] = v;
+    stream[e] = dg_stream_value(w3, w2, e);
 }
 
 __device__ __forceinline__ void dg_load_tile(const float* row, int T, f32x4 (&m)[4]) {
diff --git a/implicit_depth_amd/csrc/lidf_launch.h b/implicit_depth_amd/csrc/lidf_launch.h
--- a/implicit_depth_amd/csrc/lidf_launch.h
+++ b/implicit_depth_amd/csrc/lidf_launch.h
@@ -166,7 +166,7 @@
                                 float* dwenc, float* dbenc, float* bacc, float* scratch, hipStream_t st);
 hipError_t lidf_launch_ief_first_pass(const float* btot, float* bacc, float init, const float* w1enc, int ld1,
                                       const float* wenc, const float* benc, float* dw1enc, float* dwenc, float* dbenc,
-                                      hipStream_t st);
+                                      hipStream_t st, int clear = 0);
 hipError_t lidf_launch_build_rows(const int* pair_ray, const int* pair_vox, const float* pair_t, const float* ray_dir,
                                   const float* vox_center, int pos_rel, const float* vox_feat, const float* rayfeat,
                                   int ld_rf, int L, int Ed, long long P, float* rows, int D, hipStream_t st);
@@ -175,7 +175,7 @@
                                      hipStream_t st);
 hipError_t lidf_launch_rayfeat_backward(const float* d_rayfeat, int ld_rf, const int* ray_pix, const int* ray_bid,
                                         long long R, int half, int B, int H, int W, float* d_feat, float* gimg,
-                                        int* aux, hipStream_t st);
+                                        int* aux, hipStream_t st, int zero_d_feat = 0);
 hipError_t lidf_launch_pe_rows(const int* pair_ray, const int* pair_vox, const float* pair_t, const float* ray_dir,
                                const float* vox_center, int pos_rel, int L, long long P, float* pe, hipStream_t st,
                                const int* n_dev = nullptr, long long row0 = 0);
diff --git a/implicit_depth_amd/csrc/lidf_points.hip b/implicit_depth_amd/csrc/lidf_points.hip
--- a/implicit_depth_amd/csrc/lidf_points.hip
+++ b/implicit_depth_amd/csrc/lidf_points.hip
@@ -228,6 +228,10 @@
     if (lay.mode == LIDF_MODE_PNET_BWD) {
         const PnetW w = {net0.w1, net0.b1, net0.w2, net0.b2, net0.w3, net0.b3, net0.w4};
         if (e < lay.total) stream[e] = pn_bwd_stream_value(w, e);
+        return;
+    }
+    if (lay.mode == LIDF_MODE_DGRAD) {
+        if (e < lay.total) stream[e] = dg_stream_value(net0.w3, net0.w2, e);
         return;
     }
     if (lay.mode == LIDF_MODE_IEF16) {
diff --git a/implicit_depth_amd/csrc/lidf_train.hip b/implicit_depth_amd/csrc/lidf_train.hip
--- a/implicit_depth_amd/csrc/lidf_train.hip
+++ b/implicit_depth_amd/csrc/lidf_train.hip
@@ -682,14 +682,17 @@
 __global__ void __launch_bounds__(256) lidf_ief_finish_kernel(
     const float* __restrict__ sums, const float* __restrict__ w1enc, int ld1,
     const float* __restrict__ wenc, const float* __restrict__ benc, float* __restrict__ dw1enc,
-    float* __restrict__ dwenc, float* __restrict__ dbenc, float* __restrict__ bacc,
-    const float* __restrict__ btot, float init) {
+    float* __restrict__ dwenc, float* __restrict__ dbenc, float* bacc, const float* btot, float init, float* clear_acc) {
     __shared__ float sA[256], sB[256];
     const int c = threadIdx.x;
     float A, B;
     if (btot) {
         B = btot[c] - bacc[c];
         A = init * B;
+        if (clear_acc) {
+            clear_acc[c] = 0.f;
+            bacc[c] = 0.f;
+        }
     } else {
         A = sums[c];
         B = sums[256 + c];
@@ -756,7 +759,7 @@
     if (w1enc) {
         hipLaunchKernelGGL(lidf_colsum_reduce_kernel, dim3(32), dim3(256), 0, st, scratch, G, 512, sums);
         hipLaunchKernelGGL(lidf_ief_finish_kernel, dim3(1), dim3(256), 0, st, sums, w1enc, ld1, wenc,
-                           benc, dw1enc, dwenc, dbenc, bacc, (const float*)nullptr, 0.f);
+                           benc, dw1enc, dwenc, dbenc, bacc, (const float*)nullptr, 0.f, (float*)nullptr);
     }
     return hipGetLastError();
 }
@@ -764,9 +767,10 @@
 extern "C" hipError_t lidf_launch_ief_first_pass(const float* btot, float* bacc, float init,
                                                  const float* w1enc, int ld1, const float* wenc,
                                                  const float* benc, float* dw1enc, float* dwenc,
-                                                 float* dbenc, hipStream_t st) {
+                                                 float* dbenc, hipStream_t st, int clear) {
     hipLaunchKernelGGL(lidf_ief_finish_kernel, dim3(1), dim3(256), 0, st, (const float*)nullptr, w1enc,
-                       ld1, wenc, benc, dw1enc, dwenc, dbenc, bacc, btot, init);
+                       ld1, wenc, benc, dw1enc, dwenc, dbenc, bacc, btot, init,
+                       clear ? const_cast<float*>(btot) : (float*)nullptr);
     return hipGetLastError();
 }
 
@@ -1046,20 +1050,26 @@
                                                    const int* ray_pix, const int* ray_bid,
                                                    long long R, int half, int B, int H, int W,
                                                    float* d_feat, float* gimg, int* aux,
-                                                   hipStream_t st) {
-    if (R <= 0) return hipSuccess;
+                                                   hipStream_t st, int zero_d_feat) {
+    if (R <= 0) {
+        if (!zero_d_feat) return hipSuccess;
+        float* const zp[1] = {d_feat};
+        const long long zc[1] = {(long long)B * 32 * H * W};
+        return lidf_launch_zero_segments(zp, zc, 1, st);
+    }
     if (half <= 0) gimg = nullptr;
     const int tx_n = (W + 15) / 16, ty_n = (H + 15) / 16;
     if (!gimg || half > 16 || W < 2 * half + 1 || H < 2 * half + 1 || W - 16 * (tx_n - 1) < half ||
         H - 16 * (ty_n - 1) < half)
         aux = nullptr;
-    if (gimg) {
-        hipError_t e = hipMemsetAsync(gimg, 0, (size_t)B * 128 * H * W * 4, st);
+    {
+        float* const zp[3] = {zero_d_feat ? d_feat : nullptr, gimg, (float*)aux};
+        const long long hw = (long long)B * H * W;
+        const long long zc[3] = {32 * hw, 128 * hw, hw};
+        hipError_t e = lidf_launch_zero_segments(zp, zc, 3, st);
         if (e != hipSuccess) return e;
     }
     if (aux) {
-        hipError_t e = hipMemsetAsync(aux, 0, (size_t)B * H * W * 4, st);
-        if (e != hipSuccess) return e;
         hipLaunchKernelGGL(lidf_rayfeat_count_kernel, dim3((unsigned)((R + 255) / 256)), dim3(256), 0, st,
                            ray_pix, ray_bid, R, H, W, aux);
     }
```

Result: no change. 388.9, median of 4 (+0.1%).
